# WinnerBy/PreGANPlus

Hardware: AMD Instinct MI355X
Metric: host-windows/sec (detect+diagnose+generate) (higher is better)
Workload: dtype fp32; 1 GPU; C2: PreGAN+ batched inference, 50 hosts x W=3 x 3 resources, 65536 windows per GPU, fp32; windows_per_gpu=65536, parallelism=dp1 (independent windows)

## Files before the change

### include/preganplus.h

```cpp
#ifndef PREGANPLUS_H
#define PREGANPLUS_H

#include <stddef.h>

#ifdef __cplusplus
extern "C" {
#endif

#define PGP_ABI_VERSION 1

#define PGP_OK 0
#define PGP_ERR_ARG (-1)
#define PGP_ERR_UNSUPPORTED (-2)
#define PGP_ERR_HIP (-3)
#define PGP_ERR_STATE (-4)

typedef struct pgp_model pgp_model;

int pgp_abi_version(void);
const char* pgp_last_error(void);

int pgp_supported_hosts(int* out, int cap);

int pgp_create(int n_hosts, int n_protos, pgp_model** out);
int pgp_destroy(pgp_model* m);

size_t pgp_weight_blob_len(int n_hosts, int n_protos);

int pgp_load_weights(pgp_model* m, const double* blob, size_t len);

int pgp_reserve(pgp_model* m, int max_batch);

int pgp_forward(pgp_model* m, int batch, const float* windows, const float* sched,
                float* logits, float* protos, int* cls, int* any_anom,
                float* probs, int* keep_orig, int* final_target, int* gen_target,
                float* latent, void* stream);

int pgp_forward_stage(pgp_model* m, int stage, int batch, const float* windows,
                      const float* sched, float* logits, float* protos, int* cls,
                      int* any_anom, float* probs, int* keep_orig, int* final_target,
                      int* gen_target, float* latent, void* stream);

int pgp_migrations(int n_hosts, int batch, const int* keep_orig, const int* final_target, const int* cur_host,
                   int* moves, int* hosts_from, void* stream);
int pgp_embedding(int n_hosts, int batch, const float* logits, const float* protos, float* emb, void* stream);
int pgp_decoder_split(pgp_model* m, int on);
int pgp_encoder_split(pgp_model* m, int on);
int pgp_gan_split(pgp_model* m, int on);
int pgp_schedule_onehot(int n_hosts, int batch, const unsigned char* idx, float* sched, void* stream);

int pgp_create_fpe(int n_hosts, pgp_model** out);
size_t pgp_fpe_weight_blob_len(int n_hosts);
int pgp_forward_fpe(pgp_model* m, int batch, const float* windows, const float* h0, const float* sched,
                    float* scores, float* protos, int* cls, int* any_anom, float* probs, int* keep_orig,
                    int* final_target, int* gen_target, void* stream);
int pgp_forward_fpe_stage(pgp_model* m, int stage, int batch, const float* windows, const float* h0,
                          const float* sched, float* scores, float* protos, int* cls, int* any_anom, float* probs,
                          int* keep_orig, int* final_target, int* gen_target, void* stream);

size_t pgp_master_len(int n_hosts);
size_t pgp_tune_workspace_len(int n_hosts, int batch);
size_t pgp_gan_workspace_len(int n_hosts, int batch);
size_t pgp_master_offset(int n_hosts, int section);

int pgp_tune_forward(int n_hosts, int batch, const float* windows, const float* P, float* workspace,
                     float* latent, float* logits, float* protos, void* stream);
int pgp_tune_backward(int n_hosts, int batch, const float* P, float* G, float* workspace, const float* logits,
                      const float* protos, const int* y, const float* mult, const float* tgt, void* stream);
int pgp_tune_backward_prefix(int n_hosts, int fwd_batch, int batch, const float* P, float* G, float* workspace,
                             const float* logits, const float* protos, const int* y, const float* mult,
                             const float* tgt, void* stream);
int pgp_tune_set_side_stream(void* stream);
int pgp_tune_reserve_cus(int n);
int pgp_tune_timing(int on);
int pgp_tune_fused_ms(float* ms6);
int pgp_tune_plan_info(int n_hosts, int fwd_batch, int batch, int* out, int cap);
int pgp_gan_plan_info(int n_hosts, int batch);
int pgp_tune_targets(int n_hosts, int n_protos, const float* logits, const float* protos, const int* y, const int* cls,
                     double* state, double update_min, double decay, float* mult, float* tgt, double* loss,
                     void* stream);
int pgp_tune_step1(int n_hosts, int n_protos, const float* window, const int* y, const int* cls, const float* P,
                   float* G, double* state, double update_min, double decay, float* logits, float* protos,
                   double* loss, void* stream);
size_t pgp_tune_dropout_mask_len(int n_hosts);
int pgp_tune_step1_dropout(int n_hosts, int n_protos, const float* window, const int* y, const int* cls,
                           const float* P, float* G, double* state, double update_min, double decay, float* logits,
                           float* protos, double* loss, float p, const unsigned long long* rng_device, int step,
                           void* stream);
int pgp_tune_dropout_masks(int n_hosts, float p, const unsigned long long* rng_device, int step, unsigned char* keep,
                           void* stream);
int pgp_tune_forward_many(int n_hosts, int n_windows, const float* windows, const float* P, double* logits,
                          double* protos, void* stream);
int pgp_forward1(int n_hosts, int n_protos, const float* window, const float* sched, const float* P,
                 const double* prototypes_device, float* logits, float* protos, int* cls, int* any_anom, float* probs,
                 int* keep_orig, int* final_target, int* gen_target, void* stream);
int pgp_tune_dataset(int n_hosts, int n_env, int n_rows, const double* series, const double* train_max,
                     float* windows, int* y, int* cls, float* infer, void* stream);
size_t pgp_tune_targets_dp_workspace_len(int batch);
int pgp_tune_targets_dp(int n_hosts, int n_protos, int batch, const float* logits, const float* protos, const int* y,
                        const int* cls, const double* state, double update_min, float* mult, float* tgt, double* loss,
                        double* inc, double* workspace, void* stream);
int pgp_tune_state_apply(int n_protos, double* state, const double* inc, double decay, int n_cond,
                         const int* cond_rows, double* cond_steps, float* adam_table, double lr, double beta1,
                         double beta2, void* stream);
int pgp_gan_forward(int n_hosts, int batch, const float* emb, const float* sched, const float* P, float* workspace,
                    float* ns, float* probs, void* stream);
int pgp_gan_disc_backward(int n_hosts, int batch, const float* target, const float* P, float* G, float* workspace,
                          void* stream);
int pgp_gan_gen_backward(int n_hosts, int batch, const float* P, float* G, float* workspace, void* stream);
int pgp_gan_probs(int n_hosts, int batch, const float* workspace, float* probs, void* stream);

typedef struct {
  long long offset;
  int n;
  int active;
  float step_size;
  float bc2_sqrt;
} pgp_adam_tensor;
int pgp_adamw(float* P, const float* G, float* exp_avg, float* exp_avg_sq, float lr, float weight_decay,
              float beta1, float beta2, float eps, const pgp_adam_tensor* tensors, int ntensors, void* stream);
int pgp_adamw_table(float* P, const float* G, float* exp_avg, float* exp_avg_sq, float lr, float weight_decay,
                    float beta1, float beta2, float eps, const pgp_adam_tensor* tensors, int ntensors,
                    const float* sched, void* stream);

int pgp_gan_forward1(int n_hosts, const float* emb, const float* sched, const float* P, float* workspace, float* ns,
                     float* probs, void* stream);
int pgp_gan_step1(int n_hosts, const float* target, float* P, float* G, float* exp_avg, float* exp_avg_sq,
                  float lr_disc, float lr_gen, float weight_decay, float beta1, float beta2, float eps,
                  const pgp_adam_tensor* disc_tensors, int n_disc, const float* disc_sched,
                  const pgp_adam_tensor* gen_tensors, int n_gen, const float* gen_sched, float* workspace,
                  float* probs_gen, float* probs_after, void* stream);

typedef struct {
  long long offset;
  int n;
  int section;
  int cond;
  double step;
} pgp_online_tensor;
typedef struct {
  int n_hosts, n_env, n_rows, n_protos;
  const double* series;
  const double* train_max;
  const float* sched;
  const double* envs;
  float *P, *G, *exp_avg, *exp_avg_sq;
  float* tune_ws;
  float *logits, *protos, *windows;
  int *y, *cls;
  double* state;
  float *mult, *tgt;
  double *loss, *inc, *dp_ws;
  float* adam_rows;
  double* cond_steps;
  float *gan_ws, *ns, *probs, *emb;
  double* sim_out;
  float* target;
  const pgp_online_tensor* tensors;
  int n_tensors, n_cond;
  double lr[3];
  double weight_decay, beta1, beta2, eps, update_min, decay;
} pgp_online_desc;
typedef struct pgp_online pgp_online;
typedef int (*pgp_collective_fn)(void* user, int which, void* stream);
#define PGP_COLL_DISC_GRAD 0
#define PGP_COLL_GEN_GRAD 1
#define PGP_COLL_TUNE_GRAD 2
#define PGP_COLL_TUNE_STATE 3
#define PGP_ONLINE_NSTAGE 10
int pgp_online_create(const pgp_online_desc* desc, pgp_online** out);
int pgp_online_destroy(pgp_online* h);
int pgp_online_step(pgp_online* h, void* main_stream, void* gan_stream, pgp_collective_fn cb, void* user);
int pgp_online_timing(pgp_online* h, int on);
int pgp_online_issue_worker(pgp_online* h, int on);
int pgp_online_stage_ms(pgp_online* h, float* ms);
int pgp_online_steps(const pgp_online* h, double* steps, int n);
int pgp_online_gan_step(pgp_online* h, void* stream);

size_t pgp_fpe_param_len(int n_hosts);
int pgp_fpe_train_step(int n_hosts, int n_protos, const float* window, const float* h0, const int* y, const int* cls,
                       const float* P, float* G, double* state, double update_min, double decay, double* loss,
                       void* stream);
int pgp_fpe_forward_many(int n_hosts, int n, const float* windows, const float* h0, const float* P, double* probs,
                         double* protos, void* stream);

int pgp_load_weights_master(pgp_model* m, const float* P_device, const double* prototypes);
int pgp_repack_master(pgp_model* m, const float* P_device, const double* prototypes_device, void* stream);
int pgp_repack_master_sections(pgp_model* m, const float* P_device, const double* prototypes_device, int sections,
                               void* stream);

typedef struct pgp_gobi pgp_gobi;
size_t pgp_gobi_weight_len(int n_hosts);
int pgp_gobi_create(int n_hosts, const float* weights, size_t len, pgp_gobi** out);
int pgp_gobi_destroy(pgp_gobi* g);
const char* pgp_gobi_last_error(void);
int pgp_gobi_optimize(pgp_gobi* g, int n_env, const float* init, float* result, int* iterations,
                      float* fitness, int max_iters, float* pre, void* stream);

int pgp_gobi_train_steps(int n_hosts, int n_samples, int n, const float* feats, const float* targets,
                         const int* order, float* P, float* exp_avg, float* exp_avg_sq, long long step0,
                         double lr, double weight_decay, double beta1, double beta2, double eps, float* loss,
                         void* stream);
int pgp_gobi_train_eval(int n_hosts, int n_samples, int n, const float* feats, const float* targets,
                        const int* order, const float* P, float* loss, void* stream);

typedef struct pgp_gobi_job {
  long long sample_off, order_off;
  long long step0;
  int n_samples, n;
  double lr, weight_decay, beta1, beta2, eps;
} pgp_gobi_job;
int pgp_gobi_train_steps_many(int n_hosts, int n_models, const pgp_gobi_job* jobs, long long n_pool_samples,
                              const float* feats, const float* targets, long long n_pool_steps, const int* order,
                              float* P, float* exp_avg, float* exp_avg_sq, float* loss, void* jobs_dev,
                              void* stream);
int pgp_gobi_train_eval_many(int n_hosts, int n_models, const pgp_gobi_job* jobs, long long n_pool_samples,
                             const float* feats, const float* targets, long long n_pool_steps, const int* order,
                             const float* P, float* loss, void* jobs_dev, void* stream);

int pgp_gobi_create_many(int n_hosts, int n_models, const float* weights, size_t len, pgp_gobi** out);
int pgp_gobi_model_count(const pgp_gobi* g);
int pgp_gobi_set_model(pgp_gobi* g, int m, const float* weights, size_t len);
int pgp_gobi_optimize_groups(pgp_gobi* g, int n_env, int n_groups, const int* groups, const float* init,
                             float* result, int* iterations, float* fitness, int max_iters, float* pre,
                             void* stream);
int pgp_gobi_plan_groups(int n_env, const int* model_of_env, int n_models, int* groups_out, int cap);

size_t pgp_sim_env_len(int n_hosts);
int pgp_simulate(int n_hosts, int n_env, const double* envs, const float* new_sched, const float* orig_sched,
                 double* out, float* target, void* stream);

#ifdef __cplusplus
}
#endif

#endif
```

### preganplus_amd/_native.py

```python
from __future__ import annotations

import ctypes
import os

_HERE = os.path.dirname(os.path.abspath(__file__))
LIB_PATH = os.environ.get("PGP_LIB", os.path.join(_HERE, "_lib", "libpreganplus.so"))

PGP_OK = 0
_ERRS = {-1: "PGP_ERR_ARG", -2: "PGP_ERR_UNSUPPORTED", -3: "PGP_ERR_HIP", -4: "PGP_ERR_STATE"}

_lib = None

REMOVED_ENV = ("PGP_TUNE_SIDE_STREAM", "PGP_TUNE_SIDE_MIN_TOKENS", "PGP_TUNE_DEC_DWS", "PGP_TUNE_SIDE_EARLY",
               "PGP_TUNE_EARLY_FLUSH", "PGP_TF_SPREAD", "PGP_C3_GAN_LATE", "PGP_INIT_SEED", "PGP_SAVE_GAN_INTERVAL")


def _warn_removed_env():
    import warnings
    for k in REMOVED_ENV:
        if k in os.environ:
            hint = " (use the init_seed argument)" if k == "PGP_INIT_SEED" else ""
            warnings.warn(f"{k} is no longer read by preganplus_amd{hint}; it has no effect", RuntimeWarning,
                          stacklevel=3)


class NativeError(RuntimeError):
    pass


def lib():
    global _lib
    if _lib is not None:
        return _lib
    _warn_removed_env()
    if not os.path.exists(LIB_PATH):
        raise ImportError(
            f"HIP library not found at {LIB_PATH}; build it with `make` "
            "(hipcc --offload-arch=gfx950). There is no CPU fallback.")
    L = ctypes.CDLL(LIB_PATH)
    c_int, c_size, vp = ctypes.c_int, ctypes.c_size_t, ctypes.c_void_p
    fp = ctypes.c_void_p
    L.pgp_abi_version.argtypes = []
    L.pgp_abi_version.restype = c_int
    L.pgp_last_error.argtypes = []
    L.pgp_last_error.restype = ctypes.c_char_p
    L.pgp_supported_hosts.argtypes = [ctypes.POINTER(c_int), c_int]
    L.pgp_supported_hosts.restype = c_int
    L.pgp_weight_blob_len.argtypes = [c_int, c_int]
    L.pgp_weight_blob_len.restype = c_size
    L.pgp_create.argtypes = [c_int, c_int, ctypes.POINTER(vp)]
    L.pgp_create.restype = c_int
    L.pgp_destroy.argtypes = [vp]
    L.pgp_destroy.restype = c_int
    L.pgp_load_weights.argtypes = [vp, ctypes.POINTER(ctypes.c_double), c_size]
    L.pgp_load_weights.restype = c_int
    L.pgp_reserve.argtypes = [vp, c_int]
    L.pgp_reserve.restype = c_int
    L.pgp_forward.argtypes = [vp, c_int] + [fp] * 11 + [vp]
    L.pgp_forward.restype = c_int
    L.pgp_forward_stage.argtypes = [vp, c_int, c_int] + [fp] * 11 + [vp]
    L.pgp_forward_stage.restype = c_int
    L.pgp_create_fpe.argtypes = [c_int, ctypes.POINTER(vp)]
    L.pgp_create_fpe.restype = c_int
    L.pgp_fpe_weight_blob_len.argtypes = [c_int]
    L.pgp_fpe_weight_blob_len.restype = c_size
    L.pgp_forward_fpe.argtypes = [vp, c_int] + [fp] * 11 + [vp]
    L.pgp_forward_fpe.restype = c_int
    L.pgp_forward_fpe_stage.argtypes = [vp, c_int, c_int] + [fp] * 11 + [vp]
    L.pgp_forward_fpe_stage.restype = c_int
    L.pgp_migrations.argtypes = [c_int, c_int] + [fp] * 5 + [vp]
    L.pgp_migrations.restype = c_int
    L.pgp_embedding.argtypes = [c_int, c_int] + [fp] * 3 + [vp]
    L.pgp_embedding.restype = c_int
    L.pgp_decoder_split.argtypes = [vp, c_int]
    L.pgp_decoder_split.restype = c_int
    L.pgp_encoder_split.argtypes = [vp, c_int]
    L.pgp_encoder_split.restype = c_int
    L.pgp_gan_split.argtypes = [vp, c_int]
    L.pgp_gan_split.restype = c_int
    L.pgp_schedule_onehot.argtypes = [c_int, c_int, fp, fp, vp]
    L.pgp_schedule_onehot.restype = c_int
    _lib = L
    return L


def check(rc, what=""):
    if rc != PGP_OK:
        msg = lib().pgp_last_error().decode(errors="replace")
        raise NativeError(f"{what}: {_ERRS.get(rc, rc)}: {msg}")


def supported_hosts():
    buf = (ctypes.c_int * 16)()
    n = lib().pgp_supported_hosts(buf, 16)
    return [buf[i] for i in range(n)]
```

### preganplus_amd/csrc/pgp_capi.hip

```cpp
#include <hip/hip_runtime.h>

#include <string>

#include "../../include/preganplus.h"
#include "pgp_device.hpp"
#include "pgp_pack.hpp"
#include "pgp_repack.hpp"
#include "pgp_train.hpp"
#include "pgp_tune.hpp"
#include "pgp_tunef.hpp"
#include "pgp_tunedp.hpp"

#include <vector>

using namespace pgp;

struct pgp_model {
  int H = 0, K = 0;
  bool fpe = false;
  bool loaded = false;
  float* d_frags = nullptr;
  float* d_decb = nullptr;
  float* d_encb = nullptr;
  bool enc_split = true;
  bool dec_split = true;
  float* d_ganb = nullptr;
  bool gan_split = true;
  float* d_tab = nullptr;
  float* d_gtab = nullptr;
  float* d_gat = nullptr;
  double* d_pscr = nullptr;
  int cap = 0;
  float* d_agg = nullptr;
  float* d_lat = nullptr;
  float* d_emb = nullptr;
};

namespace {
thread_local std::string g_err;
int fail(int code, const std::string& msg) {
  g_err = msg;
  return code;
}
#define HIPCHK(x)                                                                                  \
  do {                                                                                             \
    hipError_t e_ = (x);                                                                           \
    if (e_ != hipSuccess) return fail(PGP_ERR_HIP, std::string(#x) + ": " + hipGetErrorString(e_)); \
  } while (0)

bool supported(int H) {
  switch (H) {
#define CASE(h) case h:
    PGP_FOR_EACH_H(CASE)
#undef CASE
    return true;
  }
  return false;
}

long lat_blk(int H) {
  switch (H) {
#define CASE(h) \
  case h:       \
    return Geo<h>::LAT_BLK;
    PGP_FOR_EACH_H(CASE)
#undef CASE
  }
  return 0;
}

int reserve(pgp_model* m, int n) {
  if (n <= m->cap) return PGP_OK;
  for (float** p : {&m->d_agg, &m->d_lat, &m->d_emb})
    if (*p) {
      HIPCHK(hipFree(*p));
      *p = nullptr;
    }
  m->cap = 0;
  const size_t nblk = (size_t)(n + 15) / 16;
  const size_t agg_f = m->fpe ? 4 : nblk * m->H * 3 * 48;
  const size_t lat_f = m->fpe ? 4 : nblk * (size_t)lat_blk(m->H);
  const size_t emb_f = nblk * 16 * round_up(2 * m->H, 16);
  HIPCHK(hipMalloc(&m->d_agg, agg_f * sizeof(float)));
  HIPCHK(hipMalloc(&m->d_lat, lat_f * sizeof(float)));
  HIPCHK(hipMalloc(&m->d_emb, emb_f * sizeof(float)));
  HIPCHK(hipMemset(m->d_agg, 0, agg_f * sizeof(float)));
  HIPCHK(hipMemset(m->d_lat, 0, lat_f * sizeof(float)));
  HIPCHK(hipMemset(m->d_emb, 0, emb_f * sizeof(float)));
  m->cap = n;
  return PGP_OK;
}
}

int pgp::set_error(int code, const std::string& msg) { return fail(code, msg); }

extern "C" {

int pgp_abi_version(void) { return PGP_ABI_VERSION; }
const char* pgp_last_error(void) { return g_err.c_str(); }

int pgp_supported_hosts(int* out, int cap) {
  int n = 0;
#define CASE(h)                         \
  if (out && n < cap) out[n] = h;       \
  ++n;
  PGP_FOR_EACH_H(CASE)
#undef CASE
  return n;
}

size_t pgp_weight_blob_len(int n_hosts, int n_protos) {
  if (!supported(n_hosts) || n_protos < 1) return 0;
  return blob_len(n_hosts, n_protos);
}

int pgp_create(int n_hosts, int n_protos, pgp_model** out) {
  if (!out) return fail(PGP_ERR_ARG, "out is NULL");
  *out = nullptr;
  if (!supported(n_hosts)) return fail(PGP_ERR_UNSUPPORTED, "host count not compiled in: " + std::to_string(n_hosts));
  if (n_protos < 1 || n_protos > kMaxProtos) return fail(PGP_ERR_ARG, "n_protos out of range [1,64]");
  pgp_model* m = new pgp_model();
  m->H = n_hosts;
  m->K = n_protos;
  *out = m;
  return PGP_OK;
}

size_t pgp_fpe_weight_blob_len(int n_hosts) { return fpe_blob_len(n_hosts); }

int pgp_create_fpe(int n_hosts, pgp_model** out) {
  if (!out) return fail(PGP_ERR_ARG, "out is NULL");
  *out = nullptr;
  if (fpe_blob_len(n_hosts) == 0)
    return fail(PGP_ERR_UNSUPPORTED, "FPE variant: host count not compiled in: " + std::to_string(n_hosts));
  pgp_model* m = new pgp_model();
  m->H = n_hosts;
  m->K = 3;
  m->fpe = true;
  *out = m;
  return PGP_OK;
}

int pgp_destroy(pgp_model* m) {
  if (!m) return PGP_OK;
  for (float* p : {m->d_frags, m->d_decb, m->d_encb, m->d_ganb, m->d_tab, m->d_gtab, m->d_agg, m->d_lat, m->d_emb, m->d_gat})
    if (p) (void)hipFree(p);
  if (m->d_pscr) (void)hipFree(m->d_pscr);
  delete m;
  return PGP_OK;
}

int pgp_load_weights(pgp_model* m, const double* blob, size_t len) {
  if (!m || !blob) return fail(PGP_ERR_ARG, "NULL model or blob");
  Packed P;
  const std::string err = m->fpe ? pack_fpe_weights(m->H, blob, len, &P) : pack_weights(m->H, m->K, blob, len, &P);
  if (!err.empty()) return fail(PGP_ERR_ARG, err);
  if (!m->d_frags) HIPCHK(hipMalloc(&m->d_frags, P.frags.size() * sizeof(float)));
  if (!m->d_tab) HIPCHK(hipMalloc(&m->d_tab, P.enc_tab.size() * sizeof(float)));
  if (!m->d_gtab) HIPCHK(hipMalloc(&m->d_gtab, P.gan_tab.size() * sizeof(float)));
  HIPCHK(hipMemcpy(m->d_frags, P.frags.data(), P.frags.size() * sizeof(float), hipMemcpyHostToDevice));
  HIPCHK(hipMemcpy(m->d_tab, P.enc_tab.data(), P.enc_tab.size() * sizeof(float), hipMemcpyHostToDevice));
  HIPCHK(hipMemcpy(m->d_gtab, P.gan_tab.data(), P.gan_tab.size() * sizeof(float), hipMemcpyHostToDevice));
  if (!m->d_gat) HIPCHK(hipMalloc(&m->d_gat, sizeof(GatConst)));
  HIPCHK(hipMemcpy(m->d_gat, &P.gat, sizeof(GatConst), hipMemcpyHostToDevice));
  if (!m->fpe && decoder_split_floats(m->H) > 0) {
    if (!m->d_decb) HIPCHK(hipMalloc(&m->d_decb, decoder_split_floats(m->H) * sizeof(float)));
    HIPCHK(launch_decoder_split(m->H, m->d_frags, m->d_decb, nullptr));
    HIPCHK(hipStreamSynchronize(nullptr));
  }
  if (!m->fpe && encoder_split_floats(m->H) > 0) {
    if (!m->d_encb) HIPCHK(hipMalloc(&m->d_encb, encoder_split_floats(m->H) * sizeof(float)));
    HIPCHK(launch_encoder_split(m->H, m->d_frags, m->d_encb, nullptr));
    HIPCHK(hipStreamSynchronize(nullptr));
  }
  if (gan_split_floats(m->H) > 0) {
    if (!m->d_ganb) HIPCHK(hipMalloc(&m->d_ganb, gan_split_floats(m->H) * sizeof(float)));
    HIPCHK(launch_gan_split_derive(m->H, m->d_frags, m->d_ganb, nullptr));
    HIPCHK(hipStreamSynchronize(nullptr));
  }
  m->loaded = true;
  return PGP_OK;
}

int pgp_reserve(pgp_model* m, int max_batch) {
  if (!m || max_batch < 0) return fail(PGP_ERR_ARG, "bad reserve arguments");
  return reserve(m, max_batch);
}

int pgp_forward_stage(pgp_model* m, int stage, int batch, const float* windows, const float* sched, float* logits,
                      float* protos, int* cls, int* any_anom, float* probs, int* keep_orig, int* final_target,
                      int* gen_target, float* latent, void* stream) {
  if (!m) return fail(PGP_ERR_ARG, "NULL model");
  if (!m->loaded) return fail(PGP_ERR_STATE, "weights not loaded");
  if (m->fpe) return fail(PGP_ERR_STATE, "FPE model: use pgp_forward_fpe");
  if (batch < 0) return fail(PGP_ERR_ARG, "negative batch");
  if (stage < -1 || stage > 3) return fail(PGP_ERR_ARG, "bad stage");
  if (batch == 0) return PGP_OK;
  const bool all = stage == -1;
  if (((all || stage == 0) && !windows) ||
      ((all || stage == 2) && (!logits || !protos || !cls || !any_anom)) ||
      ((all || stage == 3) && (!sched || !probs || !keep_orig || !final_target || !gen_target)))
    return fail(PGP_ERR_ARG, "NULL input/output pointer");
  if (batch > m->cap) {
    const int rc = reserve(m, batch);
    if (rc) return rc;
  }
  FwdArgs a{};
  a.B = batch;
  a.H = m->H;
  a.K = m->K;
  a.windows = windows;
  a.sched = sched;
  a.agg = m->d_agg;
  a.lat = m->d_lat;
  a.emb = m->d_emb;
  a.frags = m->d_frags;
  a.decb = m->dec_split ? m->d_decb : nullptr;
  a.encb = m->enc_split ? m->d_encb : nullptr;
  a.ganb = m->gan_split ? m->d_ganb : nullptr;
  a.tab = m->d_tab;
  a.gtab = m->d_gtab;
  a.gat = m->d_gat;
  a.logits = logits;
  a.protos = protos;
  a.cls = cls;
  a.any_anom = any_anom;
  a.probs = probs;
  a.keep = keep_orig;
  a.final_t = final_target;
  a.gen_t = gen_target;
  a.latent = latent;
  hipStream_t st = reinterpret_cast<hipStream_t>(stream);
  if (all || stage == 0) HIPCHK(launch_gat(a, st));
  if (all || stage == 1) HIPCHK(launch_encoder(a, st));
  if (all || stage == 2) HIPCHK(launch_decoder(a, st));
  if (all || stage == 3) HIPCHK(launch_gan(a, st));
  return PGP_OK;
}

int pgp_forward(pgp_model* m, int batch, const float* windows, const float* sched, float* logits, float* protos,
                int* cls, int* any_anom, float* probs, int* keep_orig, int* final_target, int* gen_target,
                float* latent, void* stream) {
  return pgp_forward_stage(m, -1, batch, windows, sched, logits, protos, cls, any_anom, probs, keep_orig,
                           final_target, gen_target, latent, stream);
}

int pgp_forward_fpe_stage(pgp_model* m, int stage, int batch, const float* windows, const float* h0,
                          const float* sched, float* scores, float* protos, int* cls, int* any_anom, float* probs,
                          int* keep_orig, int* final_target, int* gen_target, void* stream) {
  if (!m) return fail(PGP_ERR_ARG, "NULL model");
  if (!m->loaded) return fail(PGP_ERR_STATE, "weights not loaded");
  if (!m->fpe) return fail(PGP_ERR_STATE, "not an FPE model: use pgp_forward");
  if (batch < 0) return fail(PGP_ERR_ARG, "negative batch");
  if (stage < -1 || stage > 1) return fail(PGP_ERR_ARG, "bad stage");
  if (batch == 0) return PGP_OK;
  const bool all = stage == -1;
  if (((all || stage == 0) && (!windows || !h0 || !scores || !protos || !cls || !any_anom)) ||
      ((all || stage == 1) && (!sched || !probs || !keep_orig || !final_target || !gen_target)))
    return fail(PGP_ERR_ARG, "NULL input/output pointer");
  if (batch > m->cap) {
    const int rc = reserve(m, batch);
    if (rc) return rc;
  }
  hipStream_t st = reinterpret_cast<hipStream_t>(stream);
  FpeArgs f{};
  f.B = batch;
  f.windows = windows;
  f.h0 = h0;
  f.tab = m->d_tab;
  f.scores = scores;
  f.protos = protos;
  f.cls = cls;
  f.any_anom = any_anom;
  f.emb = m->d_emb;
  if (all || stage == 0) HIPCHK(launch_fpe(m->H, f, st));
  FwdArgs a{};
  a.B = batch;
  a.H = m->H;
  a.K = m->K;
  a.sched = sched;
  a.emb = m->d_emb;
  a.frags = m->d_frags;
  a.ganb = m->gan_split ? m->d_ganb : nullptr;
  a.gtab = m->d_gtab;
  a.probs = probs;
  a.keep = keep_orig;
  a.final_t = final_target;
  a.gen_t = gen_target;
  if (all || stage == 1) HIPCHK(launch_gan(a, st));
  return PGP_OK;
}

int pgp_forward_fpe(pgp_model* m, int batch, const float* windows, const float* h0, const float* sched,
                    float* scores, float* protos, int* cls, int* any_anom, float* probs, int* keep_orig,
                    int* final_target, int* gen_target, void* stream) {
  return pgp_forward_fpe_stage(m, -1, batch, windows, h0, sched, scores, protos, cls, any_anom, probs, keep_orig,
                               final_target, gen_target, stream);
}

int pgp_migrations(int n_hosts, int batch, const int* keep_orig, const int* final_target, const int* cur_host,
                   int* moves, int* hosts_from, void* stream) {
  if (n_hosts < 1 || batch < 0) return fail(PGP_ERR_ARG, "bad migrations arguments");
  if (batch == 0) return PGP_OK;
  if (!keep_orig || !final_target || !cur_host || !moves || !hosts_from)
    return fail(PGP_ERR_ARG, "NULL input/output pointer");
  HIPCHK(launch_decide(batch, n_hosts, keep_orig, final_target, cur_host, moves, hosts_from,
                       reinterpret_cast<hipStream_t>(stream)));
  return PGP_OK;
}

int pgp_embedding(int n_hosts, int batch, const float* logits, const float* protos, float* emb, void* stream) {
  if (n_hosts < 1 || batch < 0) return fail(PGP_ERR_ARG, "bad embedding arguments");
  if (batch == 0) return PGP_OK;
  if (!logits || !protos || !emb) return fail(PGP_ERR_ARG, "NULL input/output pointer");
  HIPCHK(launch_embed((long)batch * n_hosts, logits, protos, emb, reinterpret_cast<hipStream_t>(stream)));
  return PGP_OK;
}

int pgp_decoder_split(pgp_model* m, int on) {
  if (!m) return fail(PGP_ERR_ARG, "NULL model");
  if (m->fpe || decoder_split_floats(m->H) == 0)
    return on ? fail(PGP_ERR_UNSUPPORTED, "split-bf16 decoder not compiled for this model / host count") : PGP_OK;
  m->dec_split = on != 0;
  return PGP_OK;
}

int pgp_encoder_split(pgp_model* m, int on) {
  if (!m) return fail(PGP_ERR_ARG, "NULL model");
  if (m->fpe || encoder_split_floats(m->H) == 0)
    return on ? fail(PGP_ERR_UNSUPPORTED, "split-bf16 encoder not compiled for this model / host count") : PGP_OK;
  m->enc_split = on != 0;
  return PGP_OK;
}

int pgp_gan_split(pgp_model* m, int on) {
  if (!m) return fail(PGP_ERR_ARG, "NULL model");
  if (gan_split_floats(m->H) == 0)
    return on ? fail(PGP_ERR_UNSUPPORTED, "split-bf16 GAN kernel not compiled for this host count") : PGP_OK;
  m->gan_split = on != 0;
  return PGP_OK;
}

int pgp_schedule_onehot(int n_hosts, int batch, const unsigned char* idx, float* sched, void* stream) {
  if (n_hosts < 1 || n_hosts > 255 || batch < 0) return fail(PGP_ERR_ARG, "bad schedule_onehot arguments");
  if (batch == 0) return PGP_OK;
  if (!idx || !sched) return fail(PGP_ERR_ARG, "NULL input/output pointer");
  HIPCHK(launch_onehot(n_hosts, (long)batch * n_hosts, idx, sched, reinterpret_cast<hipStream_t>(stream)));
  return PGP_OK;
}

namespace {
bool master_offsets(int H, long* tr, long* gen, long* disc, long* all) {
  switch (H) {
#define CASE(h)                     \
  case h:                           \
    *tr = 0;                        \
    *gen = TGeo<h>::OFF_GEN;        \
    *disc = TGeo<h>::OFF_DISC;      \
    *all = TGeo<h>::ALL;            \
    return true;
    PGP_FOR_EACH_H(CASE)
#undef CASE
  }
  return false;
}
}

size_t pgp_master_len(int n_hosts) {
  long a, b, c, d;
  return master_offsets(n_hosts, &a, &b, &c, &d) ? (size_t)d : 0;
}
size_t pgp_master_offset(int n_hosts, int section) {
  long a, b, c, d;
  if (!master_offsets(n_hosts, &a, &b, &c, &d)) return 0;
  return section == 0 ? a : section == 1 ? b : section == 2 ? c : d;
}
size_t pgp_tune_workspace_len(int n_hosts, int batch) {
  TunePlan p;
  return (supported(n_hosts) && tune_plan(n_hosts, batch, &p)) ? (size_t)p.total : 0;
}
size_t pgp_gan_workspace_len(int n_hosts, int batch) {
  return supported(n_hosts) ? (size_t)gan_workspace_floats(n_hosts, batch) : 0;
}

int pgp_tune_forward(int n_hosts, int batch, const float* windows, const float* P, float* workspace, float* latent,
                     float* logits, float* protos, void* stream) {
  if (!supported(n_hosts)) return fail(PGP_ERR_UNSUPPORTED, "host count");
  if (batch < 0 || (batch > 0 && (!windows || !P || !workspace || !logits || !protos)))
    return fail(PGP_ERR_ARG, "bad tune_forward arguments");
  if (batch == 0) return PGP_OK;
  TunePlan p;
  tune_plan(n_hosts, batch, &p);
  HIPCHK(launch_tune_forward(p, windows, P, workspace, latent, logits, protos, reinterpret_cast<hipStream_t>(stream)));
  return PGP_OK;
}

int pgp_tune_backward(int n_hosts, int batch, const float* P, float* G, float* workspace, const float* logits,
                      const float* protos, const int* y, const float* mult, const float* tgt, void* stream) {
  if (!supported(n_hosts)) return fail(PGP_ERR_UNSUPPORTED, "host count");
  if (batch < 0 || (batch > 0 && (!P || !G || !workspace || !logits || !protos || !y || !mult || !tgt)))
    return fail(PGP_ERR_ARG, "bad tune_backward arguments");
  if (batch == 0) return PGP_OK;
  TunePlan p;
  tune_plan(n_hosts, batch, &p);
  HIPCHK(launch_tune_backward(p, P, G, workspace, logits, protos, y, mult, tgt,
                              reinterpret_cast<hipStream_t>(stream)));
  return PGP_OK;
}

int pgp_tune_backward_prefix(int n_hosts, int fwd_batch, int batch, const float* P, float* G, float* workspace,
                             const float* logits, const float* protos, const int* y, const float* mult,
                             const float* tgt, void* stream) {
  if (!supported(n_hosts)) return fail(PGP_ERR_UNSUPPORTED, "host count");
  if (batch < 0 || batch > fwd_batch ||
      (batch > 0 && (!P || !G || !workspace || !logits || !protos || !y || !mult || !tgt)))
    return fail(PGP_ERR_ARG, "bad tune_backward_prefix arguments");
  if (batch == 0) return PGP_OK;
  TunePlan p;
  if (!tune_plan_prefix(n_hosts, fwd_batch, batch, &p)) return fail(PGP_ERR_ARG, "tune_backward_prefix plan");
  HIPCHK(launch_tune_backward(p, P, G, workspace, logits, protos, y, mult, tgt,
                              reinterpret_cast<hipStream_t>(stream)));
  return PGP_OK;
}

size_t pgp_fpe_param_len(int n_hosts) { return (size_t)fpe_param_count(n_hosts); }

static const char* kFpeTrainHosts = "FPE training: n_hosts 16 or 50 only (FPE_16's architecture)";

int pgp_fpe_train_step(int n_hosts, int n_protos, const float* window, const float* h0, const int* y, const int* cls,
                       const float* P, float* G, double* state, double update_min, double decay, double* loss,
                       void* stream) {
  if (fpe_param_count(n_hosts) == 0) return fail(PGP_ERR_UNSUPPORTED, kFpeTrainHosts);
  if (n_protos < 3 || n_protos > kMaxProtos) return fail(PGP_ERR_ARG, "n_protos");
  if (!window || !h0 || !y || !cls || !P || !G || !state || !loss) return fail(PGP_ERR_ARG, "NULL argument");
  HIPCHK(launch_fpe_step(n_hosts, window, h0, y, cls, P, G, n_protos, state, update_min, decay, loss,
                         reinterpret_cast<hipStream_t>(stream)));
  return PGP_OK;
}

int pgp_fpe_forward_many(int n_hosts, int n, const float* windows, const float* h0, const float* P, double* probs,
                         double* protos, void* stream) {
  if (fpe_param_count(n_hosts) == 0) return fail(PGP_ERR_UNSUPPORTED, kFpeTrainHosts);
  if (n < 0 || (n > 0 && (!windows || !h0 || !P || !probs || !protos))) return fail(PGP_ERR_ARG, "bad arguments");
  if (n == 0) return PGP_OK;
  HIPCHK(launch_fpe_forward_many(n_hosts, n, windows, h0, P, probs, protos, reinterpret_cast<hipStream_t>(stream)));
  return PGP_OK;
}

static const char* kGobiTrainHosts = "GOBI surrogate training: only energy_latency_16 exists (16 hosts)";

int pgp_gobi_train_steps(int n_hosts, int n_samples, int n, const float* feats, const float* targets,
                         const int* order, float* P, float* exp_avg, float* exp_avg_sq, long long step0,
                         double lr, double weight_decay, double beta1, double beta2, double eps, float* loss,
                         void* stream) {
  if (!gobi_train_supported(n_hosts)) return fail(PGP_ERR_UNSUPPORTED, kGobiTrainHosts);
  if (n < 0 || n_samples < 0 || step0 < 0)
    return fail(PGP_ERR_ARG, "gobi_train_steps: negative n, n_samples or step0");
  if (!(lr > 0.0) || !(weight_decay >= 0.0) || !(eps >= 0.0) || !(beta1 >= 0.0 && beta1 < 1.0) ||
      !(beta2 >= 0.0 && beta2 < 1.0))
    return fail(PGP_ERR_ARG, "gobi_train_steps: lr > 0, weight_decay >= 0, eps >= 0, betas in [0, 1)");
  if (n == 0) return PGP_OK;
  if (!feats || !targets || !order || !P || !exp_avg || !exp_avg_sq || !loss)
    return fail(PGP_ERR_ARG, "gobi_train_steps: NULL argument");
  const GobiTrainHyper hy{lr, weight_decay, beta1, beta2, eps};
  HIPCHK(launch_gobi_train_steps(n_hosts, n_samples, n, feats, targets, order, P, exp_avg, exp_avg_sq, step0, hy,
                                 loss, reinterpret_cast<hipStream_t>(stream)));
  return PGP_OK;
}

int pgp_gobi_train_eval(int n_hosts, int n_samples, int n, const float* feats, const float* targets, const int* order,
                        const float* P, float* loss, void* stream) {
  if (!gobi_train_supported(n_hosts)) return fail(PGP_ERR_UNSUPPORTED, kGobiTrainHosts);
  if (n < 0 || n_samples < 0) return fail(PGP_ERR_ARG, "gobi_train_eval: negative n or n_samples");
  if (n == 0) return PGP_OK;
  if (!feats || !targets || !order || !P || !loss) return fail(PGP_ERR_ARG, "gobi_train_eval: NULL argument");
  HIPCHK(launch_gobi_train_eval(n_hosts, n_samples, n, feats, targets, order, P, loss,
                                reinterpret_cast<hipStream_t>(stream)));
  return PGP_OK;
}

namespace {
int gobi_jobs_check(const char* who, bool steps, int n_hosts, int n_models, const pgp_gobi_job* jobs,
                    long long n_pool_samples, long long n_pool_steps, bool* work, int* max_n) {
  const std::string w(who);
  *work = false;
  *max_n = 0;
  if (!gobi_train_supported(n_hosts)) return fail(PGP_ERR_UNSUPPORTED, kGobiTrainHosts);
  if (n_models < 0 || n_pool_samples < 0 || n_pool_steps < 0)
    return fail(PGP_ERR_ARG, w + ": negative n_models or pool size");
  if (n_models == 0) return PGP_OK;
  if (!jobs) return fail(PGP_ERR_ARG, w + ": NULL jobs");
  for (int m = 0; m < n_models; ++m) {
    const pgp_gobi_job& j = jobs[m];
    const std::string at = w + ": job " + std::to_string(m) + ": ";
    if (j.n < 0 || j.n_samples < 0 || (steps && j.step0 < 0))
      return fail(PGP_ERR_ARG, at + "negative n, n_samples or step0");
    if (steps && (!(j.lr > 0.0) || !(j.weight_decay >= 0.0) || !(j.eps >= 0.0) ||
                  !(j.beta1 >= 0.0 && j.beta1 < 1.0) || !(j.beta2 >= 0.0 && j.beta2 < 1.0)))
      return fail(PGP_ERR_ARG, at + "lr > 0, weight_decay >= 0, eps >= 0, betas in [0, 1)");
    if (j.sample_off < 0 || j.sample_off > n_pool_samples || j.n_samples > n_pool_samples - j.sample_off)
      return fail(PGP_ERR_ARG, at + "sample range outside the pool");
    if (j.order_off < 0 || j.order_off > n_pool_steps || j.n > n_pool_steps - j.order_off)
      return fail(PGP_ERR_ARG, at + "order / loss range outside the pool");
    if (j.n > 0) *work = true;
    if (j.n > *max_n) *max_n = j.n;
  }
  return PGP_OK;
}
}

int pgp_gobi_train_steps_many(int n_hosts, int n_models, const pgp_gobi_job* jobs, long long n_pool_samples,
                              const float* feats, const float* targets, long long n_pool_steps, const int* order,
                              float* P, float* exp_avg, float* exp_avg_sq, float* loss, void* jobs_dev,
                              void* stream) {
  bool work;
  int max_n;
  const int rc = gobi_jobs_check("gobi_train_steps_many", true, n_hosts, n_models, jobs, n_pool_samples,
                                 n_pool_steps, &work, &max_n);
  if (rc != PGP_OK || !work) return rc;
  if (!feats || !targets || !order || !P || !exp_avg || !exp_avg_sq || !loss || !jobs_dev)
    return fail(PGP_ERR_ARG, "gobi_train_steps_many: NULL argument");
  hipStream_t st = reinterpret_cast<hipStream_t>(stream);
  HIPCHK(hipMemcpyAsync(jobs_dev, jobs, (size_t)n_models * sizeof(pgp_gobi_job), hipMemcpyHostToDevice, st));
  HIPCHK(launch_gobi_train_steps_many(n_hosts, n_models, static_cast<const pgp_gobi_job*>(jobs_dev), feats, targets,
                                      order, P, exp_avg, exp_avg_sq, loss, st));
  return PGP_OK;
}

int pgp_gobi_train_eval_many(int n_hosts, int n_models, const pgp_gobi_job* jobs, long long n_pool_samples,
                             const float* feats, const float* targets, long long n_pool_steps, const int* order,
                             const float* P, float* loss, void* jobs_dev, void* stream) {
  bool work;
  int max_n;
  const int rc = gobi_jobs_check("gobi_train_eval_many", false, n_hosts, n_models, jobs, n_pool_samples,
                                 n_pool_steps, &work, &max_n);
  if (rc != PGP_OK || !work) return rc;
  if (!feats || !targets || !order || !P || !loss || !jobs_dev)
    return fail(PGP_ERR_ARG, "gobi_train_eval_many: NULL argument");
  hipStream_t st = reinterpret_cast<hipStream_t>(stream);
  HIPCHK(hipMemcpyAsync(jobs_dev, jobs, (size_t)n_models * sizeof(pgp_gobi_job), hipMemcpyHostToDevice, st));
  HIPCHK(launch_gobi_train_eval_many(n_hosts, n_models, max_n, static_cast<const pgp_gobi_job*>(jobs_dev), feats,
                                     targets, order, P, loss, st));
  return PGP_OK;
}

int pgp_tune_reserve_cus(int n) {
  if (n < 0) return fail(PGP_ERR_ARG, "negative CU count");
  tf_reserve_cus(n);
  return PGP_OK;
}

int pgp_tune_set_side_stream(void* stream) {
  HIPCHK(tune_set_side_stream(reinterpret_cast<hipStream_t>(stream)));
  return PGP_OK;
}

int pgp_tune_timing(int on) {
  HIPCHK(tune_timing(on != 0));
  return PGP_OK;
}

int pgp_tune_plan_info(int n_hosts, int fwd_batch, int batch, int* out, int cap) {
  if (!supported(n_hosts)) return fail(PGP_ERR_UNSUPPORTED, "host count");
  if (!out || cap < 0 || batch < 1 || batch > fwd_batch) return fail(PGP_ERR_ARG, "bad tune_plan_info arguments");
  int v[kTunePlanInfo];
  if (!tune_plan_info(n_hosts, fwd_batch, batch, v)) return fail(PGP_ERR_ARG, "tune_plan_info plan");
  for (int i = 0; i < kTunePlanInfo && i < cap; ++i) out[i] = v[i];
  return kTunePlanInfo;
}

int pgp_gan_plan_info(int n_hosts, int batch) {
  if (!supported(n_hosts)) return fail(PGP_ERR_UNSUPPORTED, "host count");
  if (batch < 1) return fail(PGP_ERR_ARG, "batch >= 1");
  const int s = gan_plan_slices(n_hosts, batch);
  return s > 0 ? s : fail(PGP_ERR_UNSUPPORTED, "host count");
}

int pgp_tune_fused_ms(float* ms6) {
  if (!ms6) return fail(PGP_ERR_ARG, "NULL output");
  const hipError_t e = tune_fused_ms(ms6);
  if (e == hipErrorInvalidValue) return fail(PGP_ERR_STATE, "pgp_tune_timing(1) was never called");
  HIPCHK(e);
  return PGP_OK;
}

int pgp_tune_targets(int n_hosts, int n_protos, const float* logits, const float* protos, const int* y, const int* cls,
                     double* state, double update_min, double decay, float* mult, float* tgt, double* loss,
                     void* stream) {
  if (n_hosts <= 0 || n_hosts > 64) return fail(PGP_ERR_UNSUPPORTED, "host count");
  if (n_protos < 3) return fail(PGP_ERR_ARG, "triplet_loss needs prototypes 0-2");
  if (!logits || !protos || !y || !cls || !state || !mult || !tgt || !loss)
    return fail(PGP_ERR_ARG, "bad tune_targets arguments");
  HIPCHK(launch_tune_targets(n_hosts, n_protos, logits, protos, y, cls, state, update_min, decay, mult, tgt, loss,
                             reinterpret_cast<hipStream_t>(stream)));
  return PGP_OK;
}

int pgp_tune_step1(int n_hosts, int n_protos, const float* window, const int* y, const int* cls, const float* P,
                   float* G, double* state, double update_min, double decay, float* logits, float* protos,
                   double* loss, void* stream) {
  if (!tune1_supported(n_hosts)) return fail(PGP_ERR_UNSUPPORTED, "host count (fused step: 8 or 16)");
  if (n_protos < 3) return fail(PGP_ERR_ARG, "triplet_loss needs prototypes 0-2");
  if (!window || !y || !cls || !P || !G || !state || !logits || !protos || !loss)
    return fail(PGP_ERR_ARG, "bad tune_step1 arguments");
  HIPCHK(launch_tune1(n_hosts, n_protos, window, y, cls, P, G, state, update_min, decay, logits, protos, loss,
                      reinterpret_cast<hipStream_t>(stream)));
  return PGP_OK;
}

size_t pgp_tune_dropout_mask_len(int n_hosts) { return tune1_dropout_mask_len(n_hosts); }

namespace {
inline bool drop_threshold(float p, unsigned int* thr) {
  if (!(p >= 0.f && p < 1.f)) return false;
  *thr = (unsigned int)((double)p * 4294967296.0);
  return true;
}
}

int pgp_tune_step1_dropout(int n_hosts, int n_protos, const float* window, const int* y, const int* cls, const float* P,
                           float* G, double* state, double update_min, double decay, float* logits, float* protos,
                           double* loss, float p, const unsigned long long* rng_device, int step, void* stream) {
  if (!tune1_supported(n_hosts)) return fail(PGP_ERR_UNSUPPORTED, "host count (fused step with dropout: 8 or 16)");
  unsigned int thr = 0;
  if (!drop_threshold(p, &thr)) return fail(PGP_ERR_ARG, "dropout p outside [0, 1)");
  if (n_protos < 3) return fail(PGP_ERR_ARG, "triplet_loss needs prototypes 0-2");
  if (!window || !y || !cls || !P || !G || !state || !logits || !protos || !loss || step < 0)
    return fail(PGP_ERR_ARG, "bad tune_step1_dropout arguments");
  hipStream_t st = reinterpret_cast<hipStream_t>(stream);
  if (thr == 0) {
    HIPCHK(launch_tune1(n_hosts, n_protos, window, y, cls, P, G, state, update_min, decay, logits, protos, loss, st));
    return PGP_OK;
  }
  if (!rng_device) return fail(PGP_ERR_ARG, "dropout needs rng_device = {seed, base step}");
  HIPCHK(launch_tune1_dropout(n_hosts, n_protos, window, y, cls, P, G, state, update_min, decay, logits, protos, loss,
                              thr, 1.0f / (1.0f - p), rng_device, step, st));
  return PGP_OK;
}

int pgp_tune_dropout_masks(int n_hosts, float p, const unsigned long long* rng_device, int step, unsigned char* keep,
                           void* stream) {
  if (!tune1_supported(n_hosts)) return fail(PGP_ERR_UNSUPPORTED, "host count (dropout masks: 8 or 16)");
  unsigned int thr = 0;
  if (!drop_threshold(p, &thr)) return fail(PGP_ERR_ARG, "dropout p outside [0, 1)");
  if (!rng_device || !keep || step < 0 || (reinterpret_cast<uintptr_t>(keep) & 3))
    return fail(PGP_ERR_ARG, "bad tune_dropout_masks arguments (keep: 4-byte aligned)");
  HIPCHK(launch_drop_masks(n_hosts, thr, rng_device, step, keep, reinterpret_cast<hipStream_t>(stream)));
  return PGP_OK;
}

int pgp_tune_forward_many(int n_hosts, int n_windows, const float* windows, const float* P, double* logits,
                          double* protos, void* stream) {
  if (!tune1_supported(n_hosts)) return fail(PGP_ERR_UNSUPPORTED, "host count (fused forward: 8 or 16)");
  if (n_windows < 0) return fail(PGP_ERR_ARG, "n_windows >= 0");
  if (n_windows == 0) return PGP_OK;
  if (!windows || !P || !logits || !protos) return fail(PGP_ERR_ARG, "bad tune_forward_many arguments");
  HIPCHK(launch_fwd_many(n_hosts, n_windows, windows, P, logits, protos, reinterpret_cast<hipStream_t>(stream)));
  return PGP_OK;
}

int pgp_forward1(int n_hosts, int n_protos, const float* window, const float* sched, const float* P,
                 const double* prototypes_device, float* logits, float* protos, int* cls, int* any_anom, float* probs,
                 int* keep_orig, int* final_target, int* gen_target, void* stream) {
  if (!tune1_supported(n_hosts)) return fail(PGP_ERR_UNSUPPORTED, "host count (batch-1 forward: 8 or 16)");
  if (n_protos < 1 || n_protos > kMaxProtos) return fail(PGP_ERR_ARG, "n_protos out of range");
  if (!window || !sched || !P || !prototypes_device || !logits || !protos || !cls || !any_anom || !probs ||
      !keep_orig || !final_target || !gen_target)
    return fail(PGP_ERR_ARG, "bad forward1 arguments");
  HIPCHK(launch_infer1(n_hosts, n_protos, window, sched, P, prototypes_device, logits, protos, cls, any_anom, probs,
                       keep_orig, final_target, gen_target, reinterpret_cast<hipStream_t>(stream)));
  return PGP_OK;
}

int pgp_tune_dataset(int n_hosts, int n_env, int n_rows, const double* series, const double* train_max,
                     float* windows, int* y, int* cls, float* infer, void* stream) {
  if (n_hosts <= 0 || n_hosts > 64) return fail(PGP_ERR_UNSUPPORTED, "host count");
  if (n_env < 0 || n_rows < 1 || n_rows > kMaxTuneRows) return fail(PGP_ERR_ARG, "n_env >= 0, 1 <= n_rows <= 16");
  if (n_env == 0) return PGP_OK;
  if (!series || !train_max || !windows || !y || !cls) return fail(PGP_ERR_ARG, "bad tune_dataset arguments");
  HIPCHK(launch_tune_dataset(n_hosts, n_env, n_rows, series, train_max, windows, y, cls, infer,
                             reinterpret_cast<hipStream_t>(stream)));
  return PGP_OK;
}

size_t pgp_tune_targets_dp_workspace_len(int batch) {
  return batch > 0 ? (size_t)tune_dp_workspace_doubles(batch) : 0;
}

int pgp_tune_targets_dp(int n_hosts, int n_protos, int batch, const float* logits, const float* protos, const int* y,
                        const int* cls, const double* state, double update_min, float* mult, float* tgt, double* loss,
                        double* inc, double* workspace, void* stream) {
  if (n_hosts <= 0 || n_hosts > 64) return fail(PGP_ERR_UNSUPPORTED, "host count");
  if (n_protos < 3 || n_protos > kMaxProtos) return fail(PGP_ERR_ARG, "triplet_loss needs prototypes 0-2");
  if (batch <= 0 || !logits || !protos || !y || !cls || !state || !mult || !tgt || !loss || !inc || !workspace)
    return fail(PGP_ERR_ARG, "bad tune_targets_dp arguments");
  HIPCHK(launch_tune_targets_dp(n_hosts, n_protos, batch, logits, protos, y, cls, const_cast<double*>(state),
                                update_min, mult, tgt, loss, inc, workspace, reinterpret_cast<hipStream_t>(stream)));
  return PGP_OK;
}

int pgp_tune_state_apply(int n_protos, double* state, const double* inc, double decay, int n_cond,
                         const int* cond_rows, double* cond_steps, float* adam_table, double lr, double beta1,
                         double beta2, void* stream) {
  if (n_protos < 3 || n_protos > kMaxProtos || !state || !inc) return fail(PGP_ERR_ARG, "bad state arguments");
  if (n_cond < 0 || n_cond > kMaxCond || (n_cond > 0 && (!cond_rows || !cond_steps || !adam_table)))
    return fail(PGP_ERR_ARG, "bad AdamW condition arguments");
  CondRows cr{};
  cr.n = n_cond;
  for (int i = 0; i < n_cond; ++i) {
    if (cond_rows[i] < 0 || cond_rows[i] >= kMaxTensors) return fail(PGP_ERR_ARG, "AdamW table row out of range");
    cr.row[i] = cond_rows[i];
  }
  HIPCHK(launch_tune_state_apply(n_protos, state, inc, decay, cr, cond_steps, adam_table, lr, beta1, beta2,
                                 reinterpret_cast<hipStream_t>(stream)));
  return PGP_OK;
}

int pgp_gan_forward(int n_hosts, int batch, const float* emb, const float* sched, const float* P, float* workspace,
                    float* ns, float* probs, void* stream) {
  long tr, go, dof, all;
  if (!master_offsets(n_hosts, &tr, &go, &dof, &all)) return fail(PGP_ERR_UNSUPPORTED, "host count");
  if (batch < 0 || (batch > 0 && (!emb || !sched || !P || !workspace || !ns || !probs)))
    return fail(PGP_ERR_ARG, "bad gan_forward arguments");
  if (batch == 0) return PGP_OK;
  HIPCHK(launch_gan_fwd(n_hosts, batch, emb, sched, P + go, P + dof, workspace, ns, probs,
                        reinterpret_cast<hipStream_t>(stream)));
  return PGP_OK;
}

int pgp_gan_disc_backward(int n_hosts, int batch, const float* target, const float* P, float* G, float* workspace,
                          void* stream) {
  long tr, go, dof, all;
  if (!master_offsets(n_hosts, &tr, &go, &dof, &all)) return fail(PGP_ERR_UNSUPPORTED, "host count");
  if (batch < 0 || (batch > 0 && (!target || !P || !G || !workspace))) return fail(PGP_ERR_ARG, "bad arguments");
  if (batch == 0) return PGP_OK;
  HIPCHK(launch_gan_disc_bwd(n_hosts, batch, target, P + dof, G + dof, workspace,
                             reinterpret_cast<hipStream_t>(stream)));
  return PGP_OK;
}

int pgp_gan_gen_backward(int n_hosts, int batch, const float* P, float* G, float* workspace, void* stream) {
  long tr, go, dof, all;
  if (!master_offsets(n_hosts, &tr, &go, &dof, &all)) return fail(PGP_ERR_UNSUPPORTED, "host count");
  if (batch < 0 || (batch > 0 && (!P || !G || !workspace))) return fail(PGP_ERR_ARG, "bad arguments");
  if (batch == 0) return PGP_OK;
  HIPCHK(launch_gan_gen_bwd(n_hosts, batch, P + go, P + dof, G + go, workspace,
                            reinterpret_cast<hipStream_t>(stream)));
  return PGP_OK;
}

int pgp_gan_forward1(int n_hosts, const float* emb, const float* sched, const float* P, float* workspace, float* ns,
                     float* probs, void* stream) {
  long tr, go, dof, all;
  if (!gan1_supported(n_hosts) || !master_offsets(n_hosts, &tr, &go, &dof, &all))
    return fail(PGP_ERR_UNSUPPORTED, "host count (fused GAN step: 8 or 16)");
  if (!emb || !sched || !P || !workspace || !ns || !probs) return fail(PGP_ERR_ARG, "bad gan_forward1 arguments");
  HIPCHK(launch_gan1_forward(n_hosts, emb, sched, P + go, P + dof, workspace, ns, probs,
                             reinterpret_cast<hipStream_t>(stream)));
  return PGP_OK;
}

static bool adam_args(AdamArgs* a, float* P, float* G, float* m, float* v, float lr, float wd, float b1, float b2,
                      float eps, const pgp_adam_tensor* t, int n, const float* sched, long lo, long hi) {
  if (!t || !sched || n < 0 || n > kMaxTensors) return false;
  *a = AdamArgs{};
  a->param = P;
  a->grad = G;
  a->m = m;
  a->v = v;
  a->lr_wd = lr * wd;
  a->b1 = b1;
  a->b2 = b2;
  a->eps = eps;
  a->ntensors = n;
  a->sched = sched;
  for (int i = 0; i < n; ++i) {
    if (t[i].offset < lo || t[i].n < 0 || (long)t[i].offset + t[i].n > hi) return false;
    a->t[i].off = (long)t[i].offset;
    a->t[i].n = t[i].n;
    a->t[i].active = 1;
  }
  return true;
}

int pgp_gan_step1(int n_hosts, const float* target, float* P, float* G, float* exp_avg, float* exp_avg_sq,
                  float lr_disc, float lr_gen, float weight_decay, float beta1, float beta2, float eps,
                  const pgp_adam_tensor* disc_tensors, int n_disc, const float* disc_sched,
                  const pgp_adam_tensor* gen_tensors, int n_gen, const float* gen_sched, float* workspace,
                  float* probs_gen, float* probs_after, void* stream) {
  long tr, go, dof, all;
  if (!gan1_supported(n_hosts) || !master_offsets(n_hosts, &tr, &go, &dof, &all))
    return fail(PGP_ERR_UNSUPPORTED, "host count (fused GAN step: 8 or 16)");
  if (!target || !P || !G || !exp_avg || !exp_avg_sq || !workspace || !probs_gen || !probs_after)
    return fail(PGP_ERR_ARG, "bad gan_step1 arguments");
  AdamArgs ad, ag;
  if (!adam_args(&ad, P, G, exp_avg, exp_avg_sq, lr_disc, weight_decay, beta1, beta2, eps, disc_tensors, n_disc,
                 disc_sched, dof, all) ||
      !adam_args(&ag, P, G, exp_avg, exp_avg_sq, lr_gen, weight_decay, beta1, beta2, eps, gen_tensors, n_gen,
                 gen_sched, go, dof))
    return fail(PGP_ERR_ARG, "AdamW tensors (disc / gen sections) or tables");
  HIPCHK(launch_gan1_step(n_hosts, target, P + go, P + dof, G + go, G + dof, workspace, ad, ag, probs_gen, probs_after,
                          reinterpret_cast<hipStream_t>(stream)));
  return PGP_OK;
}

int pgp_gan_probs(int n_hosts, int batch, const float* workspace, float* probs, void* stream) {
  if (!supported(n_hosts)) return fail(PGP_ERR_UNSUPPORTED, "host count");
  if (batch < 0 || (batch > 0 && (!workspace || !probs))) return fail(PGP_ERR_ARG, "bad arguments");
  if (batch == 0) return PGP_OK;
  HIPCHK(launch_gan_probs(n_hosts, batch, workspace, probs, reinterpret_cast<hipStream_t>(stream)));
  return PGP_OK;
}

int pgp_adamw(float* P, const float* G, float* exp_avg, float* exp_avg_sq, float lr, float weight_decay,
              float beta1, float beta2, float eps, const pgp_adam_tensor* tensors, int ntensors, void* stream) {
  if (!P || !G || !exp_avg || !exp_avg_sq || !tensors || ntensors < 0 || ntensors > kMaxTensors)
    return fail(PGP_ERR_ARG, "bad adamw arguments");
  if (ntensors == 0) return PGP_OK;
  AdamArgs a{};
  a.param = P;
  a.grad = const_cast<float*>(G);
  a.m = exp_avg;
  a.v = exp_avg_sq;
  a.lr_wd = lr * weight_decay;
  a.b1 = beta1;
  a.b2 = beta2;
  a.eps = eps;
  a.ntensors = ntensors;
  for (int i = 0; i < ntensors; ++i) {
    a.t[i].off = (long)tensors[i].offset;
    a.t[i].n = tensors[i].n;
    a.t[i].active = tensors[i].active;
    a.t[i].step_size = tensors[i].step_size;
    a.t[i].bc2_sqrt = tensors[i].bc2_sqrt;
  }
  HIPCHK(launch_adamw(a, reinterpret_cast<hipStream_t>(stream)));
  return PGP_OK;
}

int pgp_adamw_table(float* P, const float* G, float* exp_avg, float* exp_avg_sq, float lr, float weight_decay,
                    float beta1, float beta2, float eps, const pgp_adam_tensor* tensors, int ntensors,
                    const float* sched, void* stream) {
  if (!P || !G || !exp_avg || !exp_avg_sq || !tensors || !sched || ntensors < 0 || ntensors > kMaxTensors)
    return fail(PGP_ERR_ARG, "bad adamw arguments");
  if (ntensors == 0) return PGP_OK;
  AdamArgs a{};
  a.param = P;
  a.grad = const_cast<float*>(G);
  a.m = exp_avg;
  a.v = exp_avg_sq;
  a.lr_wd = lr * weight_decay;
  a.b1 = beta1;
  a.b2 = beta2;
  a.eps = eps;
  a.ntensors = ntensors;
  a.sched = sched;
  for (int i = 0; i < ntensors; ++i) {
    a.t[i].off = (long)tensors[i].offset;
    a.t[i].n = tensors[i].n;
    a.t[i].active = kAdamFromTable;
    a.t[i].step_size = tensors[i].step_size;
    a.t[i].bc2_sqrt = tensors[i].bc2_sqrt;
  }
  HIPCHK(launch_adamw(a, reinterpret_cast<hipStream_t>(stream)));
  return PGP_OK;
}

int pgp_repack_master(pgp_model* m, const float* P_device, const double* prototypes_device, void* stream) {
  return pgp_repack_master_sections(m, P_device, prototypes_device, 3, stream);
}

int pgp_repack_master_sections(pgp_model* m, const float* P_device, const double* prototypes_device, int sections,
                               void* stream) {
  if (!m || !P_device || !prototypes_device) return fail(PGP_ERR_ARG, "NULL argument");
  if (sections < 1 || sections > 3) return fail(PGP_ERR_ARG, "sections: 1 (PreGAN+), 2 (GAN) or 3 (both)");
  if (m->fpe) return fail(PGP_ERR_STATE, "FPE model: master-layout reload covers the PreGAN+ model only");
  if (!m->loaded) return fail(PGP_ERR_STATE, "weights not loaded (the first load packs on the host)");
  long tr, go, dof, all;
  if (!master_offsets(m->H, &tr, &go, &dof, &all)) return fail(PGP_ERR_UNSUPPORTED, "host count");
  if (repack_blob_protos_offset(m->H, m->K) != all) return fail(PGP_ERR_STATE, "master / blob layout mismatch");
  if (!m->d_pscr) HIPCHK(hipMalloc(&m->d_pscr, repack_scratch_len(m->H) * sizeof(double)));
  RepackArgs a{m->K, P_device, all, prototypes_device, m->d_pscr, m->d_frags, m->d_tab, m->d_gtab, m->d_gat, sections};
  HIPCHK(launch_repack(m->H, a, reinterpret_cast<hipStream_t>(stream)));
  if ((sections & 1) && m->d_decb)
    HIPCHK(launch_decoder_split(m->H, m->d_frags, m->d_decb, reinterpret_cast<hipStream_t>(stream)));
  if ((sections & 1) && m->d_encb)
    HIPCHK(launch_encoder_split(m->H, m->d_frags, m->d_encb, reinterpret_cast<hipStream_t>(stream)));
  if ((sections & 2) && m->d_ganb)
    HIPCHK(launch_gan_split_derive(m->H, m->d_frags, m->d_ganb, reinterpret_cast<hipStream_t>(stream)));
  return PGP_OK;
}

int pgp_load_weights_master(pgp_model* m, const float* P_device, const double* prototypes) {
  if (!m || !P_device || !prototypes) return fail(PGP_ERR_ARG, "NULL argument");
  if (m->fpe) return fail(PGP_ERR_STATE, "FPE model: master-layout reload covers the PreGAN+ model only");
  long tr, go, dof, all;
  if (!master_offsets(m->H, &tr, &go, &dof, &all)) return fail(PGP_ERR_UNSUPPORTED, "host count");
  std::vector<float> host((size_t)all);
  HIPCHK(hipMemcpy(host.data(), P_device, host.size() * sizeof(float), hipMemcpyDeviceToHost));
  std::vector<double> blob(host.size() + 2 * (size_t)m->K);
  for (size_t i = 0; i < host.size(); ++i) blob[i] = host[i];
  for (int k = 0; k < 2 * m->K; ++k) blob[host.size() + k] = prototypes[k];
  return pgp_load_weights(m, blob.data(), blob.size());
}

}
```

### preganplus_amd/csrc/pgp_device.hpp

```cpp
#pragma once
#include <hip/hip_runtime.h>

#include <atomic>
#include <string>

#include "pgp_layout.hpp"

struct pgp_gobi_job;

namespace pgp {

typedef float f32x4 __attribute__((ext_vector_type(4)));
typedef float f32x2 __attribute__((ext_vector_type(2)));

constexpr int kMaxProtos = 64;

inline int device_cus() {
  static std::atomic<int> cached[64];
  int dev = 0;
  if (hipGetDevice(&dev) != hipSuccess || dev < 0 || dev >= 64) return 256;
  int n = cached[dev].load(std::memory_order_relaxed);
  if (n == 0) {
    if (hipDeviceGetAttribute(&n, hipDeviceAttributeMultiprocessorCount, dev) != hipSuccess || n <= 0) n = 256;
    cached[dev].store(n, std::memory_order_relaxed);
  }
  return n;
}

struct FwdArgs {
  int B, H, K;
  const float* windows;
  const float* sched;
  float* agg;
  float* lat;
  float* emb;
  const float* frags;
  const float* decb;
  const float* ganb;
  const float* encb;
  const float* tab;
  const float* gtab;
  const float* gat;
  float* logits;
  float* protos;
  int* cls;
  int* any_anom;
  float* probs;
  int* keep;
  int* final_t;
  int* gen_t;
  float* latent;
};

struct FpeArgs {
  int B;
  const float* windows;
  const float* h0;
  const float* tab;
  float* scores;
  float* protos;
  int* cls;
  int* any_anom;
  float* emb;
};
hipError_t launch_fpe(int H, const FpeArgs& a, hipStream_t st);
int fpe_param_count(int H);
hipError_t launch_fpe_step(int n_hosts, const float* win, const float* h0, const int* y, const int* cls,
                           const float* P, float* G, int K, double* state, double update_min, double decay,
                           double* loss, hipStream_t st);
hipError_t launch_fpe_forward_many(int n_hosts, int n, const float* wins, const float* h0s, const float* P,
                                   double* probs, double* protos, hipStream_t st);

struct GobiTrainHyper {
  double lr, wd, beta1, beta2, eps;
};
bool gobi_train_supported(int H);
hipError_t launch_gobi_train_steps(int n_hosts, int n_samples, int n, const float* feats, const float* targets,
                                   const int* order, float* P, float* m, float* v, long long step0,
                                   const GobiTrainHyper& hy, float* loss, hipStream_t st);
hipError_t launch_gobi_train_eval(int n_hosts, int n_samples, int n, const float* feats, const float* targets,
                                  const int* order, const float* P, float* loss, hipStream_t st);
hipError_t launch_gobi_train_steps_many(int n_hosts, int n_models, const pgp_gobi_job* jobs_dev, const float* feats,
                                        const float* targets, const int* order, float* P, float* m, float* v,
                                        float* loss, hipStream_t st);
hipError_t launch_gobi_train_eval_many(int n_hosts, int n_models, int max_n, const pgp_gobi_job* jobs_dev,
                                       const float* feats, const float* targets, const int* order, const float* P,
                                       float* loss, hipStream_t st);

hipError_t launch_decide(int B, int C, const int* keep, const int* target, const int* cur, int* moves,
                         int* hosts_from, hipStream_t st);
hipError_t launch_embed(long n, const float* logits, const float* protos, float* emb, hipStream_t st);
hipError_t launch_onehot(int H, long rows, const unsigned char* idx, float* sched, hipStream_t st);

hipError_t launch_gat(const FwdArgs& a, hipStream_t st);
hipError_t launch_encoder(const FwdArgs& a, hipStream_t st);
hipError_t launch_decoder(const FwdArgs& a, hipStream_t st);
long decoder_split_floats(int H);
hipError_t launch_decoder_split(int H, const float* frags, float* decb, hipStream_t st);
long encoder_split_floats(int H);
hipError_t launch_encoder_split(int H, const float* frags, float* encb, hipStream_t st);
hipError_t launch_gan(const FwdArgs& a, hipStream_t st);
long gan_split_floats(int H);
hipError_t launch_gan_split_derive(int H, const float* frags, float* planes, hipStream_t st);
hipError_t launch_gan_split(const FwdArgs& a, hipStream_t st);

struct AdamArgs;
struct AdamFuse;
long gan_workspace_floats(int H, int B);
int gan_plan_slices(int H, int B);
hipError_t launch_adamw(const AdamArgs& a, hipStream_t st);
bool gan1_supported(int H);
hipError_t launch_gan1_forward(int H, const float* emb, const float* sched, const float* Pg, const float* Pd,
                               float* row, float* ns, float* probs, hipStream_t st);
hipError_t launch_gan1_step(int H, const float* target, float* Pg, float* Pd, float* Gg, float* Gd, float* row,
                            const AdamArgs& ad, const AdamArgs& ag, float* probs_gen, float* probs_after,
                            hipStream_t st);

hipError_t launch_gan_fwd(int H, int B, const float* emb, const float* sched, const float* Pg, const float* Pd,
                          float* ws, float* ns_out, float* probs, hipStream_t st, const float* logits = nullptr,
                          const float* protos = nullptr, float* emb_out = nullptr);
hipError_t launch_gan_disc_bwd(int H, int B, const float* target, const float* Pd, float* Gdd, float* ws,
                               hipStream_t st, float* probs = nullptr, const AdamFuse* af = nullptr);
hipError_t launch_gan_gen_bwd(int H, int B, const float* Pg, const float* Pd, float* Gdg, float* ws,
                              hipStream_t st, const AdamFuse* af = nullptr);
hipError_t launch_gan_probs(int H, int B, const float* ws, float* probs, hipStream_t st);
hipError_t launch_simulate(int H, int E, const double* envs, const float* new_sched, const float* orig_sched,
                           double* out, float* target, hipStream_t st);

#define PGP_DEV __device__ __forceinline__

PGP_DEV f32x4 mfma(float a, float b, f32x4 c) { return __builtin_amdgcn_mfma_f32_16x16x4f32(a, b, c, 0, 0, 0); }
typedef __bf16 bf16x8 __attribute__((ext_vector_type(8)));
typedef unsigned u32x4 __attribute__((ext_vector_type(4)));
PGP_DEV unsigned bf16_bits(float x) {
  const unsigned u = __float_as_uint(x);
  return (u + 0x7FFFu + ((u >> 16) & 1u)) >> 16;
}
PGP_DEV float bf16_val(unsigned h) { return __uint_as_float(h << 16); }
typedef __bf16 bf16x2 __attribute__((ext_vector_type(2)));
PGP_DEV unsigned bf16_pack(f32x2 x) { return __builtin_bit_cast(unsigned, __builtin_convertvector(x, bf16x2)); }
PGP_DEV f32x2 bf16_unpack(unsigned h) { return f32x2{__uint_as_float(h << 16), __uint_as_float(h & 0xFFFF0000u)}; }
PGP_DEV void split8(const float (&v)[8], u32x4 (&p)[3]) {
#pragma unroll
  for (int d = 0; d < 4; ++d) {
    const f32x2 x = {v[2 * d], v[2 * d + 1]};
    const unsigned h0 = bf16_pack(x);
    const f32x2 r1 = x - bf16_unpack(h0);
    const unsigned h1 = bf16_pack(r1);
    const f32x2 r2 = r1 - bf16_unpack(h1);
    p[0][d] = h0;
    p[1][d] = h1;
    p[2][d] = bf16_pack(r2);
  }
}
PGP_DEV f32x4 mfma_bf(u32x4 a, u32x4 b, f32x4 c) {
  return __builtin_amdgcn_mfma_f32_16x16x32_bf16(__builtin_bit_cast(bf16x8, a), __builtin_bit_cast(bf16x8, b), c, 0,
                                                 0, 0);
}
PGP_DEV void planes_ready(const u32x4 (&w)[3]) { asm volatile("" ::"v"(w[0]), "v"(w[1]), "v"(w[2])); }
PGP_DEV f32x4 mfma_bf6(const u32x4 (&w)[3], const u32x4 (&x)[3], f32x4 c) {
  c = mfma_bf(w[2], x[0], c);
  c = mfma_bf(w[1], x[1], c);
  c = mfma_bf(w[0], x[2], c);
  c = mfma_bf(w[1], x[0], c);
  c = mfma_bf(w[0], x[1], c);
  return mfma_bf(w[0], x[0], c);
}
PGP_DEV f32x4 mfma_bf3(const u32x4 (&w)[3], const u32x4 (&x)[3], f32x4 c) {
  c = mfma_bf(w[2], x[0], c);
  c = mfma_bf(w[1], x[0], c);
  return mfma_bf(w[0], x[0], c);
}

PGP_DEV bool arrive_last(unsigned* ctr, unsigned n, int* flag) {
  asm volatile("s_waitcnt vmcnt(0)" ::: "memory");
  __syncthreads();
  if (threadIdx.x == 0) {
    const bool last = __hip_atomic_fetch_add(ctr, 1u, __ATOMIC_RELAXED, __HIP_MEMORY_SCOPE_AGENT) == n - 1;
    if (last) {
      __builtin_amdgcn_fence(__ATOMIC_ACQUIRE, "agent");
      asm volatile("s_waitcnt vmcnt(0)" ::: "memory");
      __hip_atomic_store(ctr, 0u, __ATOMIC_RELAXED, __HIP_MEMORY_SCOPE_AGENT);
    }
    *flag = last;
  }
  __syncthreads();
  return *flag != 0;
}
PGP_DEV void store_wt(float* p, float v) { __hip_atomic_store(p, v, __ATOMIC_RELAXED, __HIP_MEMORY_SCOPE_AGENT); }
PGP_DEV f32x4 ld4(const float* p) { return *reinterpret_cast<const f32x4*>(p); }
PGP_DEV float tanh_fast(float x) {
  const float e = __expf(2.f * x);
  return 1.f - 2.f * __builtin_amdgcn_rcpf(e + 1.f);
}

PGP_DEV float xsum(float v, bool both) {
  const unsigned u = __float_as_uint(v);
  const auto r = __builtin_amdgcn_permlane16_swap(u, u, false, false);
  v = __uint_as_float(r[0]) + __uint_as_float(r[1]);
  if (both) {
    const unsigned u2 = __float_as_uint(v);
    const auto q = __builtin_amdgcn_permlane32_swap(u2, u2, false, false);
    v = __uint_as_float(q[0]) + __uint_as_float(q[1]);
  }
  return v;
}

PGP_DEV float pl_sum16(float a, float b) {
  const auto r = __builtin_amdgcn_permlane16_swap(__float_as_uint(a), __float_as_uint(b), false, false);
  return __uint_as_float(r[0]) + __uint_as_float(r[1]);
}
PGP_DEV float pl_sum32(float a, float b) {
  const auto r = __builtin_amdgcn_permlane32_swap(__float_as_uint(a), __float_as_uint(b), false, false);
  return __uint_as_float(r[0]) + __uint_as_float(r[1]);
}
PGP_DEV void xsum2(float& a, float& b) {
  const float s = pl_sum16(a, b);
  const unsigned su = __float_as_uint(s);
  const auto q = __builtin_amdgcn_permlane32_swap(su, su, false, false);
  const float t = __uint_as_float(q[0]) + __uint_as_float(q[1]);
  const unsigned tu = __float_as_uint(t);
  const auto p = __builtin_amdgcn_permlane16_swap(tu, tu, false, false);
  a = __uint_as_float(p[0]);
  b = __uint_as_float(p[1]);
}
PGP_DEV void xsum2_half(float& a, float& b) {
  const unsigned su = __float_as_uint(pl_sum16(a, b));
  const auto p = __builtin_amdgcn_permlane16_swap(su, su, false, false);
  a = __uint_as_float(p[0]);
  b = __uint_as_float(p[1]);
}
template <int NR>
PGP_DEV float xsum_rows(const float (&v)[NR]) {
  static_assert(NR >= 1 && NR <= 4, "at most 4 rows");
  const float s01 = pl_sum16(v[0], NR > 1 ? v[1] : 0.f);
  const float s23 = NR > 2 ? pl_sum16(v[2], NR > 3 ? v[3] : 0.f) : 0.f;
  return pl_sum32(s01, s23);
}

PGP_DEV void dma_groups(const float* __restrict__ src, float* dst, int ngroups, int wv, int nwaves, int lane) {
  for (int g = wv; g < ngroups; g += nwaves) {
    unsigned off = (unsigned)lane * 16u;
    asm volatile("" : "+v"(off));
    __builtin_amdgcn_global_load_lds(
        (const __attribute__((address_space(1))) void*)(reinterpret_cast<const char*>(src + (long)g * 256) + off),
        (__attribute__((address_space(3))) void*)(dst + g * 256), 16, 0, 0);
  }
}

int set_error(int code, const std::string& msg);

}
```

### preganplus_amd/csrc/pgp_encoder.hip

```cpp
#include "pgp_device.hpp"

namespace pgp {
namespace {

constexpr int kEncWaves = 4;
constexpr int kEnc16Waves = 4, kEnc16EU = 2;
template <int H>
constexpr bool tail_res() { return Geo<H>::TAIL; }
constexpr int kEncTailWaves = 8;
template <int H>
constexpr int enc_waves() { return H <= 16 ? kEnc16Waves : tail_res<H>() ? kEncTailWaves : kEncWaves; }
template <int H>
constexpr int NW_STAGE() { return enc_waves<H>(); }

#ifndef PGP_ENC_PIPE
#define PGP_ENC_PIPE 1
#endif
constexpr bool kEncPipe = PGP_ENC_PIPE != 0;
#ifndef PGP_ENC_PIPE_F32
#define PGP_ENC_PIPE_F32 0
#endif
constexpr bool kEncPipeF32 = PGP_ENC_PIPE_F32 != 0;

template <int H>
struct EncS {
  using G = Geo<H>;
  static constexpr int NBD = cdiv(G::KQ_D, 2);
  static constexpr int NBF = G::KQ_F / 2;
  static constexpr int F1S = G::MT_F * NBD * 3;
  static constexpr int F2S = G::MT_X * NBF * 3;
  static constexpr int FFN = F1S + F2S;
  static constexpr int L0F = 0;
  static constexpr int L1A = FFN;
  static constexpr int L1F = L1A + G::P_F1;
  static constexpr int GROUPS = L1F + FFN;
  static constexpr int STREAM = GROUPS * G::FQ;
  static constexpr long SIZE = STREAM;
};

template <int H, bool SPLIT = false>
struct EncLds {
  static constexpr bool TRES = tail_res<H>();
  static constexpr int RES0 = TRES ? Geo<H>::st_begin(Geo<H>::NST - 1) : 0;
  static constexpr int STREAM = SPLIT ? EncS<H>::STREAM : (kLayers * Geo<H>::LAYER_G - RES0) * Geo<H>::FQ;
  static constexpr bool RESIDENT = TRES || STREAM * 4 <= 32 * 1024;
  static constexpr int SLOT = Geo<H>::SLOT_G * Geo<H>::FQ;
  static constexpr int TAB = Geo<H>::t_size(kMaxProtos);
  static constexpr int TOTAL = (RESIDENT ? STREAM : 2 * SLOT) + TAB;
  static constexpr bool UNITS = TRES;
};

template <int H>
constexpr bool enc_split() {
  return tail_res<H>() && EncLds<H, true>::TOTAL * 4 + enc_waves<H>() * 144 * 4 <= 160 * 1024;
}

template <int H>
__global__ __launch_bounds__(256) void enc_split_kernel(const float* __restrict__ enc, float* __restrict__ out) {
  using G = Geo<H>;
  using S = EncS<H>;
  constexpr int T1 = G::MT_F * S::NBD, T2 = G::MT_X * S::NBF, TL = T1 + T2;
  const long f = (long)blockIdx.x * 4 + (threadIdx.x >> 6);
  const int lane = threadIdx.x & 63;
  if (f >= 2 * TL + G::P_F1) return;
  if (f >= 2 * TL) {
    const long i = f - 2 * TL;
    *reinterpret_cast<f32x4*>(out + (S::L1A + i) * 256 + lane * 4) = ld4(enc + (G::LAYER_G + i) * 256 + lane * 4);
    return;
  }
  const int l = (int)(f / TL), t = (int)(f % TL);
  const float* src = enc + (long)(l * G::LAYER_G + G::P_F1) * 256;
  long q0, q1, dst;
  const long base = l == 0 ? S::L0F : S::L1F;
  if (t < T1) {
    const int c = t / S::NBD, b = t % S::NBD;
    q0 = c * G::KQ_D + 2 * b;
    q1 = 2 * b + 1 < G::KQ_D ? q0 + 1 : -1;
    dst = base + (long)t * 3;
  } else {
    const int u = t - T1, m = u / S::NBF, b = u % S::NBF;
    q0 = G::G_F1 + m * G::KQ_F + 2 * b;
    q1 = q0 + 1;
    dst = base + S::F1S + (long)u * 3;
  }
  float v[8];
  const f32x4 x0 = ld4(src + q0 * 256 + lane * 4);
  const f32x4 x1 = q1 >= 0 ? ld4(src + q1 * 256 + lane * 4) : f32x4{0.f, 0.f, 0.f, 0.f};
#pragma unroll
  for (int e = 0; e < 4; ++e) {
    v[e] = x0[e];
    v[4 + e] = x1[e];
  }
  u32x4 p[3];
  split8(v, p);
#pragma unroll
  for (int k = 0; k < 3; ++k) *reinterpret_cast<u32x4*>(out + (dst + k) * 256 + lane * 4) = p[k];
}

template <int NT>
PGP_DEV void pair_tiles(const f32x4 (&T)[NT][3], int b, int w, float (&v)[8]) {
#pragma unroll
  for (int e = 0; e < 4; ++e) {
    v[e] = 2 * b < NT ? T[2 * b][w][e] : 0.f;
    v[4 + e] = 2 * b + 1 < NT ? T[2 * b + 1][w][e] : 0.f;
  }
}
PGP_DEV void planes_lds(const float* F, int lane, u32x4 (&w)[3]) {
#pragma unroll
  for (int k = 0; k < 3; ++k) w[k] = *reinterpret_cast<const u32x4*>(F + k * 256 + lane * 4);
}

template <int H>
PGP_DEV float relu_enc(float x) {
  if constexpr (Geo<H>::P8 || Geo<H>::TAIL)
    return __int_as_float(max(__float_as_int(x), 0));
  else
    return fmaxf(x, 0.f);
}

PGP_DEV void prio_mfma() { __builtin_amdgcn_s_setprio(1); }
PGP_DEV void prio_valu() { __builtin_amdgcn_s_setprio(0); }

template <int NM, int KQ, int KS, int NB, int NMA = NM>
PGP_DEV void gemm3(f32x4 (&acc)[NMA][3], const float* A, const f32x4 (&Bx)[NB][3], int lane) {
  static_assert(NM <= NMA, "accumulator tiles");
  prio_mfma();
#pragma unroll
  for (int m = 0; m < NM; ++m)
#pragma unroll
    for (int q4 = 0; q4 < KQ; ++q4) {
      const f32x4 a = ld4(A + (m * KQ + q4) * 256 + lane * 4);
#pragma unroll
      for (int e = 0; e < 4; ++e)
        if (4 * q4 + e < KS) {
#pragma unroll
          for (int w = 0; w < 3; ++w) acc[m][w] = mfma(a[e], Bx[q4][w][e], acc[m][w]);
        }
    }
  prio_valu();
}

template <int NM, int KQ, int KS, int NB, int NMA, int NR>
PGP_DEV void gemm3_rows(f32x4 (&acc)[NMA][3], const float* A, const f32x4 (&Bx)[NB][3], int lane,
                        float (&racc)[NR][3], const float* RW, int g) {
  static_assert(NM <= NMA, "accumulator tiles");
  prio_mfma();
  f32x4 an = ld4(A + lane * 4);
#pragma unroll
  for (int m = 0; m < NM; ++m)
#pragma unroll
    for (int q4 = 0; q4 < KQ; ++q4) {
      f32x4 a;
      if constexpr (kEncPipeF32) {
        a = an;
        if (m * KQ + q4 + 1 < NM * KQ) an = ld4(A + (m * KQ + q4 + 1) * 256 + lane * 4);
        __builtin_amdgcn_sched_barrier(0);
      } else {
        a = ld4(A + (m * KQ + q4) * 256 + lane * 4);
      }
      f32x4 rw[NR];
      if (m == 0) {
#pragma unroll
        for (int n = 0; n < NR; ++n) rw[n] = ld4(RW + ((n * KQ + q4) * 4 + g) * 4);
      }
#pragma unroll
      for (int e = 0; e < 4; ++e)
        if (4 * q4 + e < KS) {
#pragma unroll
          for (int w = 0; w < 3; ++w) {
            acc[m][w] = mfma(a[e], Bx[q4][w][e], acc[m][w]);
            if (m == 0) {
#pragma unroll
              for (int n = 0; n < NR; ++n) racc[n][w] = fmaf(rw[n][e], Bx[q4][w][e], racc[n][w]);
            }
          }
        }
    }
  prio_valu();
}

template <int NR>
PGP_DEV void rows_finish(float (&r)[NR][3]) {
  float* f = &r[0][0];
#pragma unroll
  for (int i = 0; i + 1 < 3 * NR; i += 2) xsum2(f[i], f[i + 1]);
  if constexpr ((3 * NR) % 2) f[3 * NR - 1] = xsum(f[3 * NR - 1], true);
}

template <int NR>
PGP_DEV float rows_pick(const float (&r)[NR][3], int w) {
  float v[NR];
#pragma unroll
  for (int n = 0; n < NR; ++n) v[n] = r[n][w];
  return xsum_rows<NR>(v);
}

template <int NR>
PGP_DEV void zero_rows(float (&r)[NR][3]) {
#pragma unroll
  for (int n = 0; n < NR; ++n)
#pragma unroll
    for (int w = 0; w < 3; ++w) r[n][w] = 0.f;
}

template <int H, bool AFFINE = true>
PGP_DEV void layer_norm_tiles(f32x4 (&acc)[Geo<H>::MT_D][3], f32x4 (&X)[Geo<H>::MT_D][3], const float* gam,
                              const float* bet, int g) {
  using G = Geo<H>;
  constexpr float invH = 1.0f / (float)H;
  float sum[3], mean[3], var[3];
#pragma unroll
  for (int w = 0; w < 3; ++w) {
    sum[w] = 0.f;
    float sq = 0.f;
#pragma unroll
    for (int mt = 0; mt < G::MT_D; ++mt) {
      sum[w] += (acc[mt][w][0] + acc[mt][w][1]) + (acc[mt][w][2] + acc[mt][w][3]);
#pragma unroll
      for (int r = 0; r < 4; ++r) sq = fmaf(acc[mt][w][r], acc[mt][w][r], sq);
    }
    xsum2(sum[w], sq);
    mean[w] = sum[w] * invH;
    var[w] = fmaxf(fmaf(-mean[w], mean[w], sq * invH), 0.f);
  }
#pragma unroll
  for (int w = 0; w < 3; ++w) {
    const float rstd = __builtin_amdgcn_rsqf(var[w] + 1e-5f);
    const float nm = -mean[w] * rstd;
#pragma unroll
    for (int mt = 0; mt < G::MT_D; ++mt) {
      f32x4 xn;
#pragma unroll
      for (int r = 0; r < 4; ++r) xn[r] = fmaf(acc[mt][w][r], rstd, nm);
      if constexpr (AFFINE) {
        const f32x4 ga = ld4(gam + 16 * mt + 4 * g), be = ld4(bet + 16 * mt + 4 * g);
        X[mt][w] = xn * ga + be;
      } else {
        X[mt][w] = xn;
      }
    }
  }
}

template <int H, bool SPLIT = false>
struct Ring {
  using G = Geo<H>;
  static constexpr bool RES = EncLds<H, SPLIT>::RESIDENT;
  float* cur;
  float* nxt;
  const float* enc;
  int next;
  int last;
  int wv, lane;
  PGP_DEV void issue() {
    if constexpr (RES) return;
    if (next < last) {
      const int si = next % (kLayers * G::NST), l = si / G::NST, k = si % G::NST;
      dma_groups(enc + (long)(l * G::LAYER_G + G::st_begin(k)) * G::FQ, nxt, G::st_end(k) - G::st_begin(k), wv,
                 enc_waves<H>(), lane);
    }
  }
  PGP_DEV void advance() {
    if constexpr (RES) {
      const int si = next % (kLayers * G::NST), l = si / G::NST, k = si % G::NST;
      int gi;
      if constexpr (SPLIT)
        gi = l == 0 ? EncS<H>::L0F : k == 2 ? EncS<H>::L1F : EncS<H>::L1A + G::st_begin(k);
      else
        gi = l * G::LAYER_G + G::st_begin(k) - EncLds<H>::RES0;
      cur = nxt + (gi > 0 ? gi : 0) * G::FQ;
      ++next;
      __builtin_amdgcn_sched_barrier(0);
      return;
    }
    __syncthreads();
    float* t = cur;
    cur = nxt;
    nxt = t;
    ++next;
    issue();
  }
};

template <int H>
PGP_DEV void attention(const f32x4 (&QKV)[3 * Geo<H>::TP][3], f32x4 (&O)[Geo<H>::TP][3]) {
  using G = Geo<H>;
  float pr[3][3];
  float sc9[9];
#pragma unroll
  for (int i = 0; i < 9; ++i) {
    const int w = i / 3, w2 = i % 3;
    float part = 0.f;
#pragma unroll
    for (int tp = 0; tp < G::TP; ++tp)
#pragma unroll
      for (int r = 0; r < 4; ++r) part += QKV[tp][w][r] * QKV[G::TP + tp][w2][r];
    if constexpr (G::P8)
      sc9[i] = part;
    else
      sc9[i] = xsum(part, true);
  }
  if constexpr (G::P8) {
#pragma unroll
    for (int i = 0; i < 8; i += 2) xsum2_half(sc9[i], sc9[i + 1]);
    sc9[8] = xsum(sc9[8], false);
  }
#pragma unroll
  for (int w = 0; w < 3; ++w) {
    const float* sc = sc9 + 3 * w;
    const float m = fmaxf(sc[0], fmaxf(sc[1], sc[2]));
    const float e0 = __expf(sc[0] - m), e1 = __expf(sc[1] - m), e2 = __expf(sc[2] - m);
    const float inv = __builtin_amdgcn_rcpf(e0 + e1 + e2);
    pr[w][0] = e0 * inv;
    pr[w][1] = e1 * inv;
    pr[w][2] = e2 * inv;
  }
#pragma unroll
  for (int tp = 0; tp < G::TP; ++tp)
#pragma unroll
    for (int w = 0; w < 3; ++w)
      O[tp][w] = pr[w][0] * QKV[2 * G::TP + tp][0] + pr[w][1] * QKV[2 * G::TP + tp][1] +
                 pr[w][2] * QKV[2 * G::TP + tp][2];
}

template <int H>
PGP_DEV void qkv_gemm(f32x4 (&QKV)[3 * Geo<H>::TP][3], const float* A, const float* tabqkv,
                      const f32x4 (&X)[Geo<H>::MT_D][3], int lane, int g) {
  using G = Geo<H>;
#pragma unroll
  for (int m = 0; m < 3 * G::TP; ++m) {
    const f32x4 bias = ld4(tabqkv + m * 16 + 4 * g);
#pragma unroll
    for (int w = 0; w < 3; ++w) QKV[m][w] = bias;
  }
  gemm3<3 * G::TP, G::KQ_D, G::KS_D, G::MT_D>(QKV, A, X, lane);
}

template <int H, int NM>
PGP_DEV void qkv_fold(f32x4 (&acc)[NM][3], int T0, int n, const float* tab, const float (&ba)[3], int lane, int g) {
  using G = Geo<H>;
#pragma unroll
  for (int m = 0; m < NM; ++m)
    if (m < n) {
      const float a = tab[G::T_F0 + (T0 + m) * 64 + lane];
#pragma unroll
      for (int w = 0; w < 3; ++w)
        acc[m][w] = mfma(a, ba[w], ld4(tab + G::T_F0B + (w * 3 * G::NQT + T0 + m) * 16 + 4 * g));
    }
}
template <int H>
PGP_DEV float row_fold_part(int m, int n, int w, const float* tab, const float (&ba)[3], int g) {
  using G = Geo<H>;
  const float t = tab[G::T_F0R + (m * G::SR + n) * 4 + g];
  return (g < 3 ? t : 0.f) * ba[w];
}
template <int H>
PGP_DEV float row_fold_bias(int m, int n, int w, const float* tab) {
  using G = Geo<H>;
  return tab[G::T_F0RB + w * 3 * G::SR + m * G::SR + n];
}

template <int H, bool F0, bool SPLIT>
PGP_DEV void encoder_layer_tail(f32x4 (&X)[Geo<H>::MT_D][3], Ring<H, SPLIT>& ring, const float* TL, int lane,
                                const float* tab, const float (&ba)[3], const float (&xv)[3][3]) {
  using G = Geo<H>;
  constexpr int TQ = G::TQ, SR = G::SR, HF = G::HF;
  const int g = lane >> 4;
  constexpr bool BIL = F0;
  f32x4 QK[BIL ? 1 : 2 * TQ][3];
  float qr[SR][3], kr[SR][3];
  if constexpr (BIL) {
  } else {
#pragma unroll
    for (int m = 0; m < 2 * TQ; ++m) {
      const f32x4 bias = ld4(TL + G::TL_QKV + m * 16 + 4 * g);
#pragma unroll
      for (int w = 0; w < 3; ++w) QK[m][w] = bias;
    }
    float qkr[2 * SR][3];
    zero_rows(qkr);
    gemm3_rows<2 * TQ, G::KQ_D, G::KS_D, G::MT_D, 2 * TQ, 2 * SR>(QK, ring.cur, X, lane, qkr, TL + G::TL_RQ, g);
    rows_finish(qkr);
#pragma unroll
    for (int n = 0; n < SR; ++n)
#pragma unroll
      for (int w = 0; w < 3; ++w) {
        qr[n][w] = qkr[n][w] + TL[G::TL_RQB + n];
        kr[n][w] = qkr[SR + n][w] + TL[G::TL_RQB + SR + n];
      }
  }
  ring.advance();
  float P0[3][3], P1[3][3];
  if constexpr (BIL) {
#pragma unroll
    for (int hh = 0; hh < 2; ++hh) {
      const float* SB = tab + G::T_F0S + hh * 36;
      float tk[3][3], vk[3][3];
#pragma unroll
      for (int w2 = 0; w2 < 3; ++w2) {
#pragma unroll
        for (int f = 0; f < 3; ++f)
          tk[w2][f] = fmaf(SB[3 * f + 2], xv[w2][2], fmaf(SB[3 * f + 1], xv[w2][1], fmaf(SB[3 * f], xv[w2][0], SB[9 + 3 * f + w2])));
#pragma unroll
        for (int w = 0; w < 3; ++w)
          vk[w][w2] = fmaf(SB[18 + 3 * w + 2], xv[w2][2], fmaf(SB[18 + 3 * w + 1], xv[w2][1], fmaf(SB[18 + 3 * w], xv[w2][0], SB[27 + 3 * w + w2])));
      }
#pragma unroll
      for (int w = 0; w < 3; ++w) {
        float s[3];
#pragma unroll
        for (int w2 = 0; w2 < 3; ++w2)
          s[w2] = fmaf(xv[w][2], tk[w2][2], fmaf(xv[w][1], tk[w2][1], fmaf(xv[w][0], tk[w2][0], vk[w][w2])));
        const float m = fmaxf(s[0], fmaxf(s[1], s[2]));
        const float e0 = __expf(s[0] - m), e1 = __expf(s[1] - m), e2 = __expf(s[2] - m);
        const float iv = __builtin_amdgcn_rcpf(e0 + e1 + e2);
        float(&Pw)[3][3] = hh == 0 ? P0 : P1;
        Pw[w][0] = e0 * iv;
        Pw[w][1] = e1 * iv;
        Pw[w][2] = e2 * iv;
      }
    }
  } else
#pragma unroll
  for (int w = 0; w < 3; ++w) {
    float s0[3], s1[3];
#pragma unroll
    for (int w2 = 0; w2 < 3; ++w2) {
      float a0 = 0.f, a1 = 0.f;
#pragma unroll
      for (int t = 0; t < HF; ++t)
#pragma unroll
        for (int r = 0; r < 4; ++r) {
          a0 = fmaf(QK[t][w][r], QK[TQ + t][w2][r], a0);
          a1 = fmaf(QK[HF + t][w][r], QK[TQ + HF + t][w2][r], a1);
        }
#pragma unroll
      for (int r = 0; r < 4; ++r) {
        const float pr = QK[2 * HF][w][r] * QK[TQ + 2 * HF][w2][r];
        if (4 * r + g < G::HT)
          a0 += pr;
        else
          a1 += pr;
      }
      xsum2(a0, a1);
      s0[w2] = a0;
      float t1 = a1;
#pragma unroll
      for (int n = 0; n < SR; ++n) t1 = fmaf(qr[n][w], kr[n][w2], t1);
      s1[w2] = t1;
    }
    const float m0 = fmaxf(s0[0], fmaxf(s0[1], s0[2])), m1 = fmaxf(s1[0], fmaxf(s1[1], s1[2]));
    const float e00 = __expf(s0[0] - m0), e01 = __expf(s0[1] - m0), e02 = __expf(s0[2] - m0);
    const float e10 = __expf(s1[0] - m1), e11 = __expf(s1[1] - m1), e12 = __expf(s1[2] - m1);
    const float i0 = __builtin_amdgcn_rcpf(e00 + e01 + e02), i1 = __builtin_amdgcn_rcpf(e10 + e11 + e12);
    P0[w][0] = e00 * i0;
    P0[w][1] = e01 * i0;
    P0[w][2] = e02 * i0;
    P1[w][0] = e10 * i1;
    P1[w][1] = e11 * i1;
    P1[w][2] = e12 * i1;
  }
  f32x4 acc[G::MT_D][3];
#pragma unroll
  for (int mt = 0; mt < G::MT_D; ++mt) {
    const f32x4 bo = ld4(TL + G::TL_BO + 16 * mt + 4 * g);
    if constexpr (F0) {
#pragma unroll
      for (int w = 0; w < 3; ++w) acc[mt][w] = bo + X[mt][w];
    } else {
      const f32x4 g0 = ld4(TL - G::TL_SIZE + G::TL_LN2G + 16 * mt + 4 * g);
#pragma unroll
      for (int w = 0; w < 3; ++w) acc[mt][w] = X[mt][w] * g0 + bo;
    }
  }
  if constexpr (F0) {
#pragma unroll
    for (int w = 0; w < 3; ++w) {
      const float y0 = P0[w][0] * ba[0] + P0[w][1] * ba[1] + P0[w][2] * ba[2];
      const float y1 = P1[w][0] * ba[0] + P1[w][1] * ba[1] + P1[w][2] * ba[2];
      const float p0 = g == 0 ? P0[w][0] : g == 1 ? P0[w][1] : g == 2 ? P0[w][2] : 0.f;
      const float p1 = g == 0 ? P1[w][0] : g == 1 ? P1[w][1] : g == 2 ? P1[w][2] : 0.f;
      const float bops[4] = {y0, p0, y1, p1};
#pragma unroll
      for (int k = 0; k < 4; ++k)
#pragma unroll
        for (int mt = 0; mt < G::MT_X; ++mt)
          acc[mt][w] = mfma(tab[G::T_F0O + (k * G::MT_X + mt) * 64 + lane], bops[k], acc[mt][w]);
      float ro[G::XR];
#pragma unroll
      for (int n = 0; n < G::XR; ++n) {
        const float* rw = tab + G::T_F0OR + n * 16;
        ro[n] = g < 3 ? rw[g] * y0 + rw[4 + g] * p0 + rw[8 + g] * y1 + rw[12 + g] * p1 : 0.f;
      }
      acc[G::MT_X][w][0] += xsum_rows<G::XR>(ro);
    }
    layer_norm_tiles<H, false>(acc, X, TL + G::TL_LN1G, TL + G::TL_LN1B, g);
  } else {
  f32x4 V[TQ][3];
  float vr[SR][3];
#pragma unroll
  for (int t = 0; t < TQ; ++t) {
    const f32x4 bias = ld4(TL + G::TL_QKV + (2 * TQ + t) * 16 + 4 * g);
#pragma unroll
    for (int w = 0; w < 3; ++w) V[t][w] = bias;
  }
  zero_rows(vr);
  gemm3_rows<TQ, G::KQ_D, G::KS_D, G::MT_D, TQ, SR>(V, ring.cur, X, lane, vr, TL + G::TL_RQ + 2 * SR * G::KQ_D * 16,
                                                         g);
  float vd[3];
  {
    const float vb = TL[G::TL_RQB + 2 * SR + g];
#pragma unroll
    for (int w = 0; w < 3; ++w) vd[w] = rows_pick<SR>(vr, w) + (g < SR ? vb : 0.f);
  }
  f32x4 O[TQ + 1][3];
#pragma unroll
  for (int w = 0; w < 3; ++w) {
#pragma unroll
    for (int t = 0; t < 2 * HF; ++t) {
      const float(&Pw)[3][3] = t < HF ? P0 : P1;
      O[t][w] = Pw[w][0] * V[t][0] + Pw[w][1] * V[t][1] + Pw[w][2] * V[t][2];
    }
#pragma unroll
    for (int r = 0; r < 4; ++r) {
      const bool h0 = 4 * r + g < G::HT;
      const float c0 = h0 ? P0[w][0] : P1[w][0], c1 = h0 ? P0[w][1] : P1[w][1], c2 = h0 ? P0[w][2] : P1[w][2];
      O[2 * HF][w][r] = c0 * V[2 * HF][0][r] + c1 * V[2 * HF][1][r] + c2 * V[2 * HF][2][r];
    }
    const float o3 = P1[w][0] * vd[0] + P1[w][1] * vd[1] + P1[w][2] * vd[2];
    O[TQ][w] = f32x4{o3, 0.f, 0.f, 0.f};
  }
  {
    float ro[G::XR][3];
    zero_rows(ro);
    gemm3_rows<G::MT_X, G::KQ_OT, G::KS_OT, TQ + 1, G::MT_D, G::XR>(acc, ring.cur + G::G_V * G::FQ, O, lane, ro,
                                                                   TL + G::TL_RO, g);
#pragma unroll
    for (int w = 0; w < 3; ++w) acc[G::MT_X][w][0] += rows_pick<G::XR>(ro, w);
  }
  layer_norm_tiles<H, false>(acc, X, TL + G::TL_LN1G, TL + G::TL_LN1B, g);
  }
  ring.advance();
#pragma unroll
  for (int mt = 0; mt < G::MT_D; ++mt) {
    const f32x4 b2 = ld4(TL + G::TL_B2 + 16 * mt + 4 * g), g1 = ld4(TL + G::TL_LN1G + 16 * mt + 4 * g);
#pragma unroll
    for (int w = 0; w < 3; ++w) acc[mt][w] = X[mt][w] * g1 + b2;
  }
  if constexpr (SPLIT) {
    using S = EncS<H>;
    static_assert(S::NBF * 2 == G::MT_F, "hidden pairs");
    const float* A1 = ring.cur;
    const float* A2 = ring.cur + S::F1S * G::FQ;
#pragma unroll
    for (int w = 0; w < 3; ++w) {
      f32x4 F[G::MT_F];
#pragma unroll
      for (int c = 0; c < G::MT_F; ++c) F[c] = ld4(TL + G::TL_B1 + 16 * c + 4 * g);
      if constexpr (kEncPipe) {
        constexpr int QN = S::NBD * G::MT_F;
        u32x4 wn[3];
        planes_lds(A1, lane, wn);
#pragma unroll
        for (int b = 0; b < S::NBD; ++b) {
          u32x4 xb[3];
          {
            float v[8];
            pair_tiles<G::MT_D>(X, b, w, v);
            split8(v, xb);
          }
          prio_mfma();
#pragma unroll
          for (int c = 0; c < G::MT_F; ++c) {
            u32x4 wp[3];
#pragma unroll
            for (int k = 0; k < 3; ++k) wp[k] = wn[k];
            const int q = b * G::MT_F + c + 1;
            if (q < QN) planes_lds(A1 + (((q % G::MT_F) * S::NBD + q / G::MT_F) * 3) * 256, lane, wn);
            __builtin_amdgcn_sched_barrier(0);
            F[c] = mfma_bf6(wp, xb, F[c]);
          }
          prio_valu();
        }
      } else {
        u32x4 xs[S::NBD][3];
#pragma unroll
        for (int b = 0; b < S::NBD; ++b) {
          float v[8];
          pair_tiles<G::MT_D>(X, b, w, v);
          split8(v, xs[b]);
        }
        prio_mfma();
#pragma unroll
        for (int b = 0; b < S::NBD; ++b)
#pragma unroll
          for (int c = 0; c < G::MT_F; ++c) {
            u32x4 wp[3];
            planes_lds(A1 + ((c * S::NBD + b) * 3) * 256, lane, wp);
            F[c] = mfma_bf6(wp, xs[b], F[c]);
          }
        prio_valu();
      }
#pragma unroll
      for (int c = 0; c < G::MT_F; ++c)
#pragma unroll
        for (int r = 0; r < 4; ++r) F[c][r] = relu_enc<H>(F[c][r]);
      float rf[G::XR];
#pragma unroll
      for (int n = 0; n < G::XR; ++n) rf[n] = 0.f;
#pragma unroll
      for (int c = 0; c < G::MT_F; ++c)
#pragma unroll
        for (int n = 0; n < G::XR; ++n) {
          const f32x4 rw = ld4(TL + G::TL_RF + ((n * G::KQ_F + c) * 4 + g) * 4);
#pragma unroll
          for (int e = 0; e < 4; ++e) rf[n] = fmaf(rw[e], F[c][e], rf[n]);
        }
      if constexpr (kEncPipe) {
        constexpr int QN = S::NBF * G::MT_X;
        u32x4 wn[3];
        planes_lds(A2, lane, wn);
#pragma unroll
        for (int b = 0; b < S::NBF; ++b) {
          u32x4 hb[3];
          {
            float v[8];
#pragma unroll
            for (int e = 0; e < 4; ++e) {
              v[e] = F[2 * b][e];
              v[4 + e] = F[2 * b + 1][e];
            }
            split8(v, hb);
          }
          prio_mfma();
#pragma unroll
          for (int m = 0; m < G::MT_X; ++m) {
            u32x4 wp[3];
#pragma unroll
            for (int k = 0; k < 3; ++k) wp[k] = wn[k];
            const int q = b * G::MT_X + m + 1;
            if (q < QN) planes_lds(A2 + (((q % G::MT_X) * S::NBF + q / G::MT_X) * 3) * 256, lane, wn);
            __builtin_amdgcn_sched_barrier(0);
            acc[m][w] = mfma_bf6(wp, hb, acc[m][w]);
          }
          prio_valu();
        }
      } else {
        u32x4 hs[S::NBF][3];
#pragma unroll
        for (int b = 0; b < S::NBF; ++b) {
          float v[8];
#pragma unroll
          for (int e = 0; e < 4; ++e) {
            v[e] = F[2 * b][e];
            v[4 + e] = F[2 * b + 1][e];
          }
          split8(v, hs[b]);
        }
        prio_mfma();
#pragma unroll
        for (int b = 0; b < S::NBF; ++b)
#pragma unroll
          for (int m = 0; m < G::MT_X; ++m) {
            u32x4 wp[3];
            planes_lds(A2 + ((m * S::NBF + b) * 3) * 256, lane, wp);
            acc[m][w] = mfma_bf6(wp, hs[b], acc[m][w]);
          }
        prio_valu();
      }
      acc[G::MT_X][w][0] += xsum_rows<G::XR>(rf);
    }
  } else {
    static_assert(G::KQ_F == G::MT_F, "hidden tile c = W2 k-group c");
    float rf[G::XR][3];
    zero_rows(rf);
#pragma unroll
    for (int c = 0; c < G::MT_F; ++c) {
      f32x4 Fc[1][3];
      const f32x4 b1 = ld4(TL + G::TL_B1 + 16 * c + 4 * g);
#pragma unroll
      for (int w = 0; w < 3; ++w) Fc[0][w] = b1;
      gemm3<1, G::KQ_D, G::KS_D, G::MT_D>(Fc, ring.cur + c * G::KQ_D * 256, X, lane);
#pragma unroll
      for (int w = 0; w < 3; ++w)
#pragma unroll
        for (int r = 0; r < 4; ++r) Fc[0][w][r] = relu_enc<H>(Fc[0][w][r]);
      const float* A2 = ring.cur + G::G_F1 * G::FQ;
      prio_mfma();
#pragma unroll
      for (int m = 0; m < G::MT_X; ++m) {
        const f32x4 a = ld4(A2 + (m * G::KQ_F + c) * 256 + lane * 4);
#pragma unroll
        for (int e = 0; e < 4; ++e)
#pragma unroll
          for (int w = 0; w < 3; ++w) acc[m][w] = mfma(a[e], Fc[0][w][e], acc[m][w]);
      }
      prio_valu();
#pragma unroll
      for (int n = 0; n < G::XR; ++n) {
        const f32x4 rw = ld4(TL + G::TL_RF + ((n * G::KQ_F + c) * 4 + g) * 4);
#pragma unroll
        for (int e = 0; e < 4; ++e)
#pragma unroll
          for (int w = 0; w < 3; ++w) rf[n][w] = fmaf(rw[e], Fc[0][w][e], rf[n][w]);
      }
    }
#pragma unroll
    for (int w = 0; w < 3; ++w) acc[G::MT_X][w][0] += rows_pick<G::XR>(rf, w);
  }
  ring.advance();
  layer_norm_tiles<H, false>(acc, X, TL + G::TL_LN2G, TL + G::TL_LN2B, g);
}

template <int H, bool F0>
PGP_DEV void encoder_layer(f32x4 (&X)[Geo<H>::MT_D][3], Ring<H>& ring, const float* TL, int lane,
                           const float* tab, const float (&ba)[3]) {
  using G = Geo<H>;
  const int g = lane >> 4;
  f32x4 acc[G::MT_D][3];
  f32x4 QKV[3 * G::TP][3];
  f32x4 O[G::TP][3];
  if constexpr (F0)
    qkv_fold<H, 3 * G::TP>(QKV, 0, 3 * G::TP, tab, ba, lane, g);
  else
    qkv_gemm<H>(QKV, ring.cur, TL + G::TL_QKV, X, lane, g);
  ring.advance();
  attention<H>(QKV, O);
#pragma unroll
  for (int mt = 0; mt < G::MT_D; ++mt) {
    const f32x4 bo = ld4(TL + G::TL_BO + 16 * mt + 4 * g);
    if constexpr (F0) {
#pragma unroll
      for (int w = 0; w < 3; ++w) acc[mt][w] = bo + X[mt][w];
    } else {
      const f32x4 g0 = ld4(TL - G::TL_SIZE + G::TL_LN2G + 16 * mt + 4 * g);
#pragma unroll
      for (int w = 0; w < 3; ++w) acc[mt][w] = X[mt][w] * g0 + bo;
    }
  }
  gemm3<G::MT_D, G::KQ_O, G::KS_O, G::TP>(acc, ring.cur, O, lane);
  if constexpr (G::NPASS == 2) {
    if constexpr (F0)
      qkv_fold<H, 3 * G::TP>(QKV, 3 * G::TP, 3 * G::TP, tab, ba, lane, g);
    else
      qkv_gemm<H>(QKV, ring.cur + G::G_O * G::FQ, TL + G::TL_QKV + 3 * G::TP * 16, X, lane, g);
    ring.advance();
    attention<H>(QKV, O);
    gemm3<G::MT_D, G::KQ_O, G::KS_O, G::TP>(acc, ring.cur, O, lane);
  }
  layer_norm_tiles<H, false>(acc, X, TL + G::TL_LN1G, TL + G::TL_LN1B, g);
  f32x4 F1[G::MT_F][3];
#pragma unroll
  for (int mt = 0; mt < G::MT_F; ++mt) {
    const f32x4 b1 = ld4(TL + G::TL_B1 + 16 * mt + 4 * g);
#pragma unroll
    for (int w = 0; w < 3; ++w) F1[mt][w] = b1;
  }
  gemm3<G::MT_F, G::KQ_D, G::KS_D, G::MT_D>(F1, ring.cur + G::G_O * G::FQ, X, lane);
#pragma unroll
  for (int mt = 0; mt < G::MT_F; ++mt)
#pragma unroll
    for (int w = 0; w < 3; ++w)
#pragma unroll
      for (int r = 0; r < 4; ++r) F1[mt][w][r] = relu_enc<H>(F1[mt][w][r]);
  ring.advance();
#pragma unroll
  for (int mt = 0; mt < G::MT_D; ++mt) {
    const f32x4 b2 = ld4(TL + G::TL_B2 + 16 * mt + 4 * g), g1 = ld4(TL + G::TL_LN1G + 16 * mt + 4 * g);
#pragma unroll
    for (int w = 0; w < 3; ++w) acc[mt][w] = X[mt][w] * g1 + b2;
  }
  gemm3<G::MT_D, G::KQ_F, 16, G::MT_F>(acc, ring.cur, F1, lane);
  ring.advance();
  layer_norm_tiles<H, false>(acc, X, TL + G::TL_LN2G, TL + G::TL_LN2B, g);
}

template <int H, bool SPLIT>
__global__ __launch_bounds__(enc_waves<H>() * 64, H <= 16 ? kEnc16EU : tail_res<H>() ? 1 : 2) void encoder_kernel(
    FwdArgs a) {
  using G = Geo<H>;
  using L = EncLds<H, SPLIT>;
  __shared__ __attribute__((aligned(16))) float smem[L::TOTAL];
  __shared__ float xstage[L::UNITS ? NW_STAGE<H>() * 144 : 1];
  float* tab = smem + (L::RESIDENT ? L::STREAM : 2 * L::SLOT);
  const int tsz = G::t_size(a.K);
  for (int i = threadIdx.x; i < tsz; i += blockDim.x) tab[i] = a.tab[i];

  const int lane = threadIdx.x & 63, g = lane >> 4, j = lane & 15;
  const int wv = __builtin_amdgcn_readfirstlane(threadIdx.x >> 6);
  constexpr int NW = enc_waves<H>();
  const long nblk = (a.B + 15) / 16;

  Ring<H, SPLIT> ring{smem, smem + L::SLOT, a.frags + G::OFF_ENC, 0, H * kLayers * G::NST, wv, lane};
  if constexpr (SPLIT) {
    dma_groups(a.encb, smem, EncS<H>::GROUPS, wv, NW, lane);
    ring.nxt = smem;
    ring.next = 1;
    __syncthreads();
  } else if constexpr (L::RESIDENT) {
    dma_groups(a.frags + G::OFF_ENC + (long)L::RES0 * G::FQ, smem, kLayers * G::LAYER_G - L::RES0, wv, NW, lane);
    ring.nxt = smem;
    ring.next = 1;
    __syncthreads();
  } else {
    ring.nxt = smem;
    ring.issue();
    ring.nxt = smem + L::SLOT;
    ring.next = 1;
    __syncthreads();
    ring.issue();
  }

  auto unit = [&](long blk, int h, bool active, const float* pre) {
    const float* agg = a.agg + (active ? blk : 0) * H * 3 * 48;
    float* lat = a.lat + (active ? blk : 0) * G::LAT_BLK;
    float ba[3];
    float xv[3][3];
    if constexpr (L::UNITS) {
#pragma unroll
      for (int w = 0; w < 3; ++w) {
#pragma unroll
        for (int f = 0; f < 3; ++f) xv[w][f] = G::TAIL ? pre[w * 48 + 16 * f + j] : 0.f;
        const float v = pre[w * 48 + (lane < 48 ? lane : 47)];
        ba[w] = g < 3 ? v : 0.f;
      }
    } else {
#pragma unroll
      for (int w = 0; w < 3; ++w) ba[w] = (active && g < 3) ? agg[(h * 3 + w) * 48 + lane] : 0.f;
#pragma unroll
      for (int w = 0; w < 3; ++w)
#pragma unroll
        for (int f = 0; f < 3; ++f)
          xv[w][f] = (G::TAIL && active) ? agg[(h * 3 + w) * 48 + 16 * f + j] : 0.f;
    }
    f32x4 X[G::MT_D][3];
#pragma unroll
    for (int mt = 0; mt < G::MT_D; ++mt) {
      const float aw = tab[G::T_TEW + mt * 64 + lane];
#pragma unroll
      for (int w = 0; w < 3; ++w) X[mt][w] = mfma(aw, ba[w], ld4(tab + G::T_TE + w * G::DP + 16 * mt + 4 * g));
    }
    static_assert(kLayers == 2, "layer 0 (folded q/k/v) + layer 1");
    if constexpr (G::TAIL) {
      encoder_layer_tail<H, true, SPLIT>(X, ring, tab + G::T_L0, lane, tab, ba, xv);
      encoder_layer_tail<H, false, SPLIT>(X, ring, tab + G::T_L0 + G::TL_SIZE, lane, tab, ba, xv);
    } else if constexpr (!SPLIT) {
      encoder_layer<H, true>(X, ring, tab + G::T_L0, lane, tab, ba);
      encoder_layer<H, false>(X, ring, tab + G::T_L0 + G::TL_SIZE, lane, tab, ba);
    }

    if (active) {
#pragma unroll
      for (int w = 0; w < 3; ++w) {
        float* lc = lat + (long)((h * 3 + w) * G::KS_D) * 64;
#pragma unroll
        for (int q = 0; q < G::LAT_FG; ++q) *reinterpret_cast<f32x4*>(lc + q * 256 + lane * 4) = X[q][w];
        if constexpr (G::KS_D % 4 != 0) {
#pragma unroll
          for (int r = 0; r < G::KS_D % 4; ++r) lc[G::LAT_FG * 256 + r * 64 + lane] = X[G::LAT_FG][w][r];
        }
      }
      if (a.latent != nullptr) {
        const long b = blk * 16 + j;
        if (b < a.B) {
#pragma unroll
          for (int w = 0; w < 3; ++w)
#pragma unroll
            for (int mt = 0; mt < G::MT_D; ++mt)
#pragma unroll
              for (int r = 0; r < 4; ++r) {
                const int c = 16 * mt + 4 * r + g;
                const float* TL1 = tab + G::T_L0 + G::TL_SIZE;
                if (c < H)
                  a.latent[b * G::LAT + (long)h * 3 * H + w * H + c] =
                      X[mt][w][r] * TL1[G::TL_LN2G + 16 * mt + 4 * g + r] + TL1[G::TL_LN2B + 16 * mt + 4 * g + r];
              }
        }
      }
    }
  };
  if constexpr (L::UNITS) {
    const long U = nblk * H, NWT = (long)gridDim.x * NW, gw = (long)blockIdx.x * NW + wv;
    const long u1 = (gw + 1) * U / NWT;
    float* slot = xstage + wv * 144;
    const long u0 = gw * U / NWT;
    float pf[3];
    auto load_x = [&](long u) {
#pragma unroll
      for (int k = 0; k < 3; ++k) pf[k] = a.agg[u * 144 + (64 * k + lane < 144 ? 64 * k + lane : 143)];
    };
    auto stage_x = [&]() {
#pragma unroll
      for (int k = 0; k < 3; ++k)
        if (64 * k + lane < 144) slot[64 * k + lane] = pf[k];
    };
    if (u0 < u1) {
      load_x(u0);
      stage_x();
    }
#pragma unroll 1
    for (long u = u0; u < u1; ++u) {
      load_x(u + 1 < u1 ? u + 1 : u);
      const long blk = u / H;
      unit(blk, (int)(u - blk * H), true, slot);
      stage_x();
    }
  } else {
    const long blk = (long)blockIdx.x * NW + wv;
    const bool active = blk < nblk;
#pragma unroll 1
    for (int h = 0; h < H; ++h) unit(blk, h, active, nullptr);
  }
}

template <int H, bool SPLIT>
hipError_t launch_form(const FwdArgs& a, hipStream_t st) {
  const long nblk = (a.B + 15) / 16;
  constexpr int NW = enc_waves<H>();
  long grid = (nblk + NW - 1) / NW;
  static std::atomic<int> fits{-1};
  if (fits.load(std::memory_order_relaxed) < 0) {
    hipFuncAttributes fa{};
    const bool ok = hipFuncGetAttributes(&fa, reinterpret_cast<const void*>(encoder_kernel<H, SPLIT>)) == hipSuccess &&
                    fa.maxThreadsPerBlock >= NW * 64;
    fits.store(ok ? 1 : 0, std::memory_order_relaxed);
  }
  if (!fits.load(std::memory_order_relaxed)) return hipErrorLaunchOutOfResources;
  if constexpr (EncLds<H>::UNITS) {
    static std::atomic<int> occ_cache{0};
    int occ = occ_cache.load(std::memory_order_relaxed);
    if (occ <= 0) {
      if (hipOccupancyMaxActiveBlocksPerMultiprocessor(&occ, encoder_kernel<H, SPLIT>, NW * 64, 0) != hipSuccess ||
          occ <= 0)
        occ = 1;
      occ_cache.store(occ, std::memory_order_relaxed);
    }
    grid = std::min<long>((long)device_cus() * occ, (nblk * H + NW - 1) / NW);
  }
  encoder_kernel<H, SPLIT><<<(int)grid, NW * 64, 0, st>>>(a);
  return hipGetLastError();
}

template <int H>
hipError_t launch(const FwdArgs& a, hipStream_t st) {
  if constexpr (enc_split<H>())
    if (a.encb != nullptr) return launch_form<H, true>(a, st);
  return launch_form<H, false>(a, st);
}

template <int H>
hipError_t launch_split(const float* frags, float* encb, hipStream_t st) {
  if constexpr (enc_split<H>()) {
    using G = Geo<H>;
    constexpr long n = 2L * (G::MT_F * EncS<H>::NBD + G::MT_X * EncS<H>::NBF) + G::P_F1;
    enc_split_kernel<H><<<(int)((n + 3) / 4), 256, 0, st>>>(frags + G::OFF_ENC, encb);
    return hipGetLastError();
  }
  return hipErrorInvalidValue;
}

}

hipError_t launch_encoder(const FwdArgs& a, hipStream_t st) {
  switch (a.H) {
#define CASE(h) \
  case h:       \
    return launch<h>(a, st);
    PGP_FOR_EACH_H(CASE)
#undef CASE
  }
  return hipErrorInvalidValue;
}

long encoder_split_floats(int H) {
  switch (H) {
#define CASE(h) \
  case h:       \
    return enc_split<h>() ? EncS<h>::SIZE : 0;
    PGP_FOR_EACH_H(CASE)
#undef CASE
  }
  return 0;
}

hipError_t launch_encoder_split(int H, const float* frags, float* encb, hipStream_t st) {
  switch (H) {
#define CASE(h) \
  case h:       \
    return launch_split<h>(frags, encb, st);
    PGP_FOR_EACH_H(CASE)
#undef CASE
  }
  return hipErrorInvalidValue;
}

}
```

### preganplus_amd/model.py

```python
from __future__ import annotations

import ctypes

import numpy as np
import torch

from . import _native
from . import weights as W


class DecisionModel:
    def __init__(self, n_hosts: int, weights: dict, device: str | torch.device = "cuda"):
        self.H = int(n_hosts)
        self.K = int(np.asarray(weights["prototypes"]).shape[0])
        self.device = torch.device(device)
        if self.device.type == "cuda" and self.device.index is None:
            self.device = torch.device("cuda", torch.cuda.current_device())
        if self.device.type != "cuda":
            raise ValueError("DecisionModel runs on the GPU only (no CPU fallback)")
        L = _native.lib()
        if self.H not in _native.supported_hosts():
            raise ValueError(f"H={self.H} not compiled in; supported {_native.supported_hosts()}")
        self._L = L
        h = ctypes.c_void_p()
        _native.check(L.pgp_create(self.H, self.K, ctypes.byref(h)), "pgp_create")
        self._h = h
        self.load_weights(weights)

    def load_weights(self, weights: dict):
        blob = W.pack_blob(weights, self.H)
        n = self._L.pgp_weight_blob_len(self.H, self.K)
        if n != blob.size:
            raise ValueError(f"blob length {blob.size} != {n}")
        torch.cuda.set_device(self.device)
        _native.check(self._L.pgp_load_weights(
            self._h, blob.ctypes.data_as(ctypes.POINTER(ctypes.c_double)), blob.size),
            "pgp_load_weights")
        self.prototypes = np.asarray(weights["prototypes"], dtype=np.float64)

    def load_master(self, P: torch.Tensor, prototypes):
        pr = np.ascontiguousarray(np.asarray(prototypes, dtype=np.float64))
        L = self._L
        L.pgp_load_weights_master.argtypes = [ctypes.c_void_p, ctypes.c_void_p, ctypes.POINTER(ctypes.c_double)]
        torch.cuda.synchronize(self.device)
        _native.check(L.pgp_load_weights_master(self._h, ctypes.c_void_p(P.data_ptr()),
                                                pr.ctypes.data_as(ctypes.POINTER(ctypes.c_double))),
                      "pgp_load_weights_master")
        self.prototypes = pr.copy()

    def repack_master(self, P: torch.Tensor, protos_dev: torch.Tensor, prototypes_host=None, stream=None,
                      sections: int = 3):
        if protos_dev.dtype != torch.float64 or protos_dev.numel() != 2 * self.K or not protos_dev.is_contiguous():
            raise ValueError(f"protos_dev must be contiguous float64 [{self.K},2] on the device")
        L = self._L
        L.pgp_repack_master_sections.argtypes = [ctypes.c_void_p] * 3 + [ctypes.c_int, ctypes.c_void_p]
        st = stream if stream is not None else torch.cuda.current_stream(self.device)
        _native.check(L.pgp_repack_master_sections(self._h, ctypes.c_void_p(P.data_ptr()),
                                                   ctypes.c_void_p(protos_dev.data_ptr()), int(sections),
                                                   ctypes.c_void_p(st.cuda_stream)), "pgp_repack_master_sections")
        if prototypes_host is not None:
            self.prototypes = np.array(prototypes_host, dtype=np.float64)

    def reserve(self, max_batch: int):
        _native.check(self._L.pgp_reserve(self._h, int(max_batch)), "pgp_reserve")

    def gan_split(self, on: bool):
        _native.check(self._L.pgp_gan_split(self._h, int(bool(on))), "pgp_gan_split")

    def encoder_split(self, on: bool):
        _native.check(self._L.pgp_encoder_split(self._h, int(bool(on))), "pgp_encoder_split")

    def decoder_split(self, on: bool):
        _native.check(self._L.pgp_decoder_split(self._h, int(bool(on))), "pgp_decoder_split")

    def alloc_outputs(self, B: int, latent: bool = False, packed: bool = False):
        dev, H = self.device, self.H
        f32, i32 = torch.float32, torch.int32
        spec = [("logits", f32, (B, H, 2)), ("protos", f32, (B, H, 2)), ("cls", i32, (B, H)), ("any", i32, (B,)),
                ("probs", f32, (B, 2)), ("keep", i32, (B,)), ("final_target", i32, (B, H)),
                ("gen_target", i32, (B, H))]
        if packed:
            n = sum(int(np.prod(s)) for _, _, s in spec)
            buf = torch.zeros(n, dtype=i32, device=dev)
            out, o = {}, 0
            for name, dt, shp in spec:
                k = int(np.prod(shp))
                out[name] = buf[o:o + k].view(dt).view(shp)
                o += k
            out["_buf"] = buf
            out["_hbuf"] = torch.zeros(n, dtype=i32).pin_memory()
        else:
            out = {name: torch.empty(shp, dtype=dt, device=dev) for name, dt, shp in spec}
        out["latent"] = torch.empty((B, 3 * H * H), dtype=f32, device=dev) if latent else None
        return out

    def _check_inputs(self, windows, sched):
        H = self.H
        B = windows.shape[0]
        if tuple(windows.shape) != (B, 3, 3 * H) or windows.dtype != torch.float32:
            raise ValueError(f"windows must be float32 [B,3,{3 * H}], got {tuple(windows.shape)} {windows.dtype}")
        if sched is not None and (tuple(sched.shape) != (B, H, H) or sched.dtype != torch.float32):
            raise ValueError(f"sched must be float32 [B,{H},{H}], got {tuple(sched.shape)} {sched.dtype}")
        for t in (windows, sched):
            if t is not None and (t.device != self.device or not t.is_contiguous()):
                raise ValueError("inputs must be contiguous tensors on the model's device")
        return B

    def forward(self, windows: torch.Tensor, sched: torch.Tensor, out: dict | None = None,
                latent: bool = False, stage: int = -1, stream=None) -> dict:
        B = self._check_inputs(windows, sched)
        if out is None:
            out = self.alloc_outputs(B, latent)
        st = stream if stream is not None else torch.cuda.current_stream(self.device)
        p = lambda t: None if t is None else t.data_ptr()
        _native.check(self._L.pgp_forward_stage(
            self._h, int(stage), B, p(windows), p(sched), p(out["logits"]), p(out["protos"]),
            p(out["cls"]), p(out["any"]), p(out["probs"]), p(out["keep"]),
            p(out["final_target"]), p(out["gen_target"]), p(out.get("latent")),
            ctypes.c_void_p(st.cuda_stream)), "pgp_forward")
        return out

    def close(self):
        if getattr(self, "_h", None) is not None and self._h.value:
            self._L.pgp_destroy(self._h)
            self._h = None

    def __del__(self):
        try:
            self.close()
        except Exception:
            pass


class FPEDecisionModel(DecisionModel):

    def __init__(self, n_hosts: int, weights: dict, device: str | torch.device = "cuda"):
        self.H = int(n_hosts)
        self.K = W.FPE_PROTOS
        self.device = torch.device(device)
        if self.device.type == "cuda" and self.device.index is None:
            self.device = torch.device("cuda", torch.cuda.current_device())
        if self.device.type != "cuda":
            raise ValueError("FPEDecisionModel runs on the GPU only (no CPU fallback)")
        L = _native.lib()
        self._L = L
        h = ctypes.c_void_p()
        _native.check(L.pgp_create_fpe(self.H, ctypes.byref(h)), "pgp_create_fpe")
        self._h = h
        self.load_weights(weights)

    def load_weights(self, weights: dict):
        if "fpe" not in weights:
            raise ValueError("FPE weights need an 'fpe' section (PreGAN FPE_16 state_dict)")
        blob = W.pack_blob(weights, self.H)
        n = self._L.pgp_fpe_weight_blob_len(self.H)
        if n != blob.size:
            raise ValueError(f"blob length {blob.size} != {n}")
        torch.cuda.set_device(self.device)
        _native.check(self._L.pgp_load_weights(
            self._h, blob.ctypes.data_as(ctypes.POINTER(ctypes.c_double)), blob.size), "pgp_load_weights")
        self.prototypes = np.asarray(weights["prototypes"], dtype=np.float64)

    def load_master(self, P, prototypes):
        raise NotImplementedError("the PreGAN encoder is frozen (PreGAN.py:29); reload GAN weights with load_weights")

    def alloc_outputs(self, B: int, latent: bool = False):
        out = super().alloc_outputs(B, False)
        out["scores"] = out.pop("logits")
        return out

    def forward(self, windows: torch.Tensor, h0: torch.Tensor, sched: torch.Tensor, out: dict | None = None,
                stage: int = -1, stream=None) -> dict:
        B = self._check_inputs(windows, sched)
        if tuple(h0.shape) != (B, 3) or h0.dtype != torch.float32 or h0.device != self.device \
                or not h0.is_contiguous():
            raise ValueError(f"h0 must be contiguous float32 [B,3] on {self.device}")
        if out is None:
            out = self.alloc_outputs(B)
        st = stream if stream is not None else torch.cuda.current_stream(self.device)
        p = lambda t: t.data_ptr()
        _native.check(self._L.pgp_forward_fpe_stage(
            self._h, int(stage), B, p(windows), p(h0), p(sched), p(out["scores"]), p(out["protos"]), p(out["cls"]),
            p(out["any"]), p(out["probs"]), p(out["keep"]), p(out["final_target"]), p(out["gen_target"]),
            ctypes.c_void_p(st.cuda_stream)), "pgp_forward_fpe")
        return out


def migrations(keep_orig: torch.Tensor, final_target: torch.Tensor, cur_host: torch.Tensor, stream=None,
               out=None):
    B, C = final_target.shape
    for t, shp in ((keep_orig, (B,)), (final_target, (B, C)), (cur_host, (B, C))):
        if tuple(t.shape) != shp or t.dtype != torch.int32 or not t.is_cuda or not t.is_contiguous():
            raise ValueError("migrations: int32 contiguous device tensors keep [B], final_target/cur_host [B,C]")
    moves, hosts_from = out if out is not None else (torch.empty_like(final_target), torch.empty_like(final_target))
    st = stream if stream is not None else torch.cuda.current_stream(final_target.device)
    _native.check(_native.lib().pgp_migrations(
        C, B, keep_orig.data_ptr(), final_target.data_ptr(), cur_host.data_ptr(), moves.data_ptr(),
        hosts_from.data_ptr(), ctypes.c_void_p(st.cuda_stream)), "pgp_migrations")
    return moves, hosts_from


def embedding(logits: torch.Tensor, protos: torch.Tensor, out: torch.Tensor | None = None, stream=None):
    B, H = logits.shape[0], logits.shape[1]
    for t in (logits, protos):
        if tuple(t.shape) != (B, H, 2) or t.dtype != torch.float32 or not t.is_cuda or not t.is_contiguous():
            raise ValueError("embedding: fp32 contiguous device tensors logits / protos [B,H,2]")
    out = torch.empty_like(protos) if out is None else out
    st = stream if stream is not None else torch.cuda.current_stream(logits.device)
    _native.check(_native.lib().pgp_embedding(H, B, logits.data_ptr(), protos.data_ptr(), out.data_ptr(),
                                              ctypes.c_void_p(st.cuda_stream)), "pgp_embedding")
    return out


def assemble_decision(original_decision, moves_row, cur_host_row):
    decision = dict(original_decision)
    moves_row = [int(v) for v in moves_row]
    cur = [int(v) for v in cur_host_row]
    order = sorted((h, c) for c, h in enumerate(cur) if h >= 0)
    for _, c in order:
        if moves_row[c] >= 0:
            decision[c] = moves_row[c]
    return list(decision.items())


def to_numpy(out: dict) -> dict:
    res = {}
    if "_buf" in out:
        hb = out["_hbuf"]
        hb.copy_(out["_buf"], non_blocking=True)
        torch.cuda.current_stream(out["_buf"].device).synchronize()
        a, o = hb.numpy(), 0
        for k, v in out.items():
            if k.startswith("_") or v is None or k == "latent":
                continue
            n = v.numel()
            x = a[o:o + n].view(np.float32 if v.dtype == torch.float32 else np.int32).reshape(tuple(v.shape)).copy()
            res[k] = x.astype(bool) if k in ("any", "keep") else x
            o += n
        if out.get("latent") is not None:
            res["latent"] = out["latent"].detach().cpu().numpy()
        return res
    for k, v in out.items():
        if v is None or k.startswith("_"):
            continue
        a = v.detach().cpu().numpy()
        if k in ("any", "keep"):
            a = a.astype(bool)
        res[k] = a
    return res
```

### preganplus_amd/roofline.py

```python
from __future__ import annotations

PEAK_FP32_TFLOPS = 157.3
PEAK_HBM_GBS = 8000.0
PEAK_BF16_TFLOPS = 2500.0

W = 3
FF = 64
GAN_HIDDEN = 64


def macs_per_window(H: int) -> dict:
    d = H
    tokens = W * H
    hd = d // 2
    gat = tokens * 3 * d + 2 * tokens * d + W * H * H * d
    te = tokens * d * d
    per_token_layer = 3 * d * d + d * d + 2 * (W * hd) * 2 + 2 * FF * d
    layers = 2 * tokens * per_token_layer
    dec = (W * H * d) * (4 * H)
    gan = GAN_HIDDEN * (2 * H + H * H) + (H * H) * GAN_HIDDEN + GAN_HIDDEN * 2 * H * H + 2 * GAN_HIDDEN
    return dict(gat=gat, time_encoder=te, encoder_layers=layers, decoders=dec, gan=gan)


def flops_per_window(H: int) -> dict:
    return {k: 2 * v for k, v in macs_per_window(H).items()}


def total_flops_per_window(H: int) -> int:
    return sum(flops_per_window(H).values())


def encdec_flops_per_window(H: int) -> int:
    f = flops_per_window(H)
    return f["time_encoder"] + f["encoder_layers"] + f["decoders"]


def encoder_flops_per_window(H: int) -> int:
    f = flops_per_window(H)
    return f["time_encoder"] + f["encoder_layers"]


ENC_MFMA_PER_HOST = {16: 264, 50: 1116}


def encoder_executed_flops_per_window(H: int):
    n = ENC_MFMA_PER_HOST.get(H)
    return None if n is None else n * 2048 * H / 16


ENC_SPLIT_MFMA_PER_HOST = {50: (516, 504)}


def encoder_split(H: int) -> bool:
    return H in ENC_SPLIT_MFMA_PER_HOST


def encoder_split_executed_flops_per_window(H: int):
    f32, bf = ENC_SPLIT_MFMA_PER_HOST[H]
    return f32 * 2048 * H / 16, bf * 16 * 16 * 32 * 2 * H / 16


TUNE_MFMA_PER_UNIT = {
    16: {"tf_fwd_kernel": 156, "tf_bwd_ffn_kernel": 288, "tf_bwd_att_kernel": 96},
    50: {"tf_fwd_kernel": 840, "tf_bwd_ffn_kernel": 384, "tf_bwd_att_kernel": 1200},
}
TUNE_BF16_PER_UNIT = {
    16: {"tf_fwd_kernel": 0, "tf_bwd_ffn_kernel": 0, "tf_bwd_att_kernel": 0},
    50: {"tf_fwd_kernel": 288, "tf_bwd_ffn_kernel": 576, "tf_bwd_att_kernel": 144},
}
TUNE_FUSED_LAUNCHES = ("fwd layer 0", "fwd layer 1", "ffn bwd layer 1", "att bwd layer 1", "ffn bwd layer 0",
                       "att bwd layer 0")


def tf_grid(units: int, waves: int, cus: int, reserve: int = 0) -> int:
    r = max(0, min(reserve, cus // 2))
    gmax = max(1, min(cus - r, (units + waves - 1) // waves))
    m = (units + waves * gmax - 1) // (waves * gmax)
    return max(1, (units + waves * m - 1) // (waves * m))


def tune_fused_grids(H: int, B: int, B_fwd: int | None, cus: int, reserve: int = 0):
    units = (B * H + 15) // 16
    ufwd = ((B if B_fwd is None else B_fwd) * H + 15) // 16
    gf, gb = tf_grid(ufwd, 8, cus, reserve), tf_grid(units, 4, cus, reserve)
    return [gf, gf, gb, gb, gb, gb]


def tune_te_mfma(H: int) -> int:
    nt = (H + 15) // 16
    ks = 4 * (H // 16) + (min(H % 16, 4) if H % 16 else 0)
    return nt * ks * 3


def tune_fused_flops(H: int, B: int, B_fwd: int | None = None):
    c = TUNE_MFMA_PER_UNIT.get(H)
    if c is None:
        return None
    bf = TUNE_BF16_PER_UNIT.get(H, {})
    eq = {k: n * 2048 + bf.get(k, 0) * 16 * 16 * 32 * 2 * PEAK_FP32_TFLOPS / PEAK_BF16_TFLOPS for k, n in c.items()}
    units = (B * H + 15) // 16
    ufwd = ((B if B_fwd is None else B_fwd) * H + 15) // 16
    fwd, te = eq["tf_fwd_kernel"], tune_te_mfma(H) * 2048
    return ([ufwd * fwd, ufwd * (fwd - te)]
            + [units * n for n in (eq["tf_bwd_ffn_kernel"], eq["tf_bwd_att_kernel"], eq["tf_bwd_ffn_kernel"],
                                   eq["tf_bwd_att_kernel"])])


def encoder_io_bytes_per_window(H: int) -> int:
    return 4 * (W * H * 3) + 4 * (W * H * H)


def decoder_flops_per_window(H: int) -> int:
    return flops_per_window(H)["decoders"]


def decoder_split(H: int) -> bool:
    return H in (32, 50)


def gan_split(H: int) -> bool:
    return H in (16, 50)


def gan_split_flops_per_window(H: int, onehot: bool = True) -> int:
    ep = (2 * H + 15) // 16
    npe = (ep + 1) // 2
    nps = ((H * H + 15) // 16 + 1) // 2
    mtn = (H + 15) // 16
    npn = (mtn + 1) // 2
    n = npe * 4 * 6 + nps * 8 * (3 if onehot else 6) + H * (mtn * 2 * 6 + 4 * npn * 6)
    return n * 16 * 16 * 32 * 2 // 16


def decoder_split_flops_per_window(H: int) -> int:
    ks = (H + 3) // 4
    nb = ((ks + 3) // 4 + 1) // 2
    mt = (4 * H + 15) // 16
    return H * W * nb * mt * 6 * 16 * 16 * 32 * 2 // 16


def gan_flops_per_window(H: int) -> int:
    return flops_per_window(H)["gan"]


def path_bytes_per_window(H: int) -> int:
    return 36 * H + 4 * H * H + 8 * H + 8 * H + 4 * H + 4 * H + 8


def fpe_macs_per_window(H: int = 16) -> int:
    E, L = H + 3, 10
    gru = W * (9 * 3 * H + 9 * 3)
    gat = W * (H * 3 * H + 2 * H * H + H * H * H)
    mha = W * 3 * E * E + 2 * W * W * E + W * E * E
    enc = W * E * L * H
    dec = H * (2 * L + 2 * L)
    return gru + gat + mha + enc + dec


def fpe_flops_per_window(H: int = 16) -> int:
    return 2 * fpe_macs_per_window(H)


def fpe_executed_flops_per_window(H: int = 16) -> int:
    per_step = H * (27 + 6) * 2 + 27 * 2 + H * H * (2 + 4) + H * (3 + 3 + 2) * 2
    mha = 3 * (36 + 6) * 2 + 9 * 6 * 2 + 3 * 3 * 6 * 2
    out = 4 * H * 18 * 2
    return 3 * per_step + mha + out


def fpe_bytes_per_window(H: int = 16) -> int:
    return 36 * H + 12 + 8 * H + 8 * H + 4 * H + 4 + 8 * H


def tune_step_flops_per_window(H: int) -> int:
    f = flops_per_window(H)
    return 3 * (f["gat"] + f["time_encoder"] + f["encoder_layers"] + f["decoders"])


def gan_step_macs_per_env(H: int, hidden: int = GAN_HIDDEN) -> int:
    gin, hh = 2 * H + H * H, H * H
    fwd = hidden * gin + hh * hidden + hidden * 2 * hh + 2 * hidden
    disc_step = 2 * hidden + 2 * hidden + hidden * 2 * hh
    gen_step = hidden * 2 * hh + 2 * hidden + 2 * hidden + 3 * hh * hidden + hidden * gin
    return fwd + disc_step + gen_step


def gan_step_flops_per_env(H: int) -> int:
    return 2 * gan_step_macs_per_env(H)
```

Baseline: 647.2 million host-windows/s.

## Add attention-split bf16 encoder form with LDS-resident pre-split weight triples

Adds a third encoder form that pre-splits the attention Q/K/V and output-projection weights into bf16 triples, alongside the existing split feed-forward weights. It makes this form the default when the split buffer exists. The Q/K/V and output GEMMs run as bf16x3 MFMA with software-pipelined plane loads, reading mostly from LDS with one streamed triple from global memory. The goal is to replace fp32 MFMA in attention with cheaper split-bf16 MFMA. In exchange it uses more LDS, which may lower occupancy, and adds register pressure and extra split-weight preparation.

```diff
diff --git a/include/preganplus.h b/include/preganplus.h
--- a/include/preganplus.h
+++ b/include/preganplus.h
@@ -46,6 +46,7 @@
 int pgp_embedding(int n_hosts, int batch, const float* logits, const float* protos, float* emb, void* stream);
 int pgp_decoder_split(pgp_model* m, int on);
 int pgp_encoder_split(pgp_model* m, int on);
+int pgp_encoder_form_info(int n_hosts, int* compiled, int* lds_bytes, int* resident_triples, int* streamed_triples);
 int pgp_gan_split(pgp_model* m, int on);
 int pgp_schedule_onehot(int n_hosts, int batch, const unsigned char* idx, float* sched, void* stream);
 
diff --git a/preganplus_amd/_native.py b/preganplus_amd/_native.py
--- a/preganplus_amd/_native.py
+++ b/preganplus_amd/_native.py
@@ -76,6 +76,9 @@
     L.pgp_decoder_split.restype = c_int
     L.pgp_encoder_split.argtypes = [vp, c_int]
     L.pgp_encoder_split.restype = c_int
+    if hasattr(L, "pgp_encoder_form_info"):
+        L.pgp_encoder_form_info.argtypes = [c_int] + [ctypes.POINTER(c_int)] * 4
+        L.pgp_encoder_form_info.restype = c_int
     L.pgp_gan_split.argtypes = [vp, c_int]
     L.pgp_gan_split.restype = c_int
     L.pgp_schedule_onehot.argtypes = [c_int, c_int, fp, fp, vp]
diff --git a/preganplus_amd/csrc/pgp_capi.hip b/preganplus_amd/csrc/pgp_capi.hip
--- a/preganplus_amd/csrc/pgp_capi.hip
+++ b/preganplus_amd/csrc/pgp_capi.hip
@@ -11,6 +11,10 @@
 #include "pgp_tunef.hpp"
 #include "pgp_tunedp.hpp"
 
+#ifndef PGP_ENC_FORM
+#define PGP_ENC_FORM 1
+#endif
+
 #include <vector>
 
 using namespace pgp;
@@ -22,7 +26,7 @@
   float* d_frags = nullptr;
   float* d_decb = nullptr;
   float* d_encb = nullptr;
-  bool enc_split = true;
+  int enc_form = PGP_ENC_FORM;
   bool dec_split = true;
   float* d_ganb = nullptr;
   bool gan_split = true;
@@ -216,7 +220,8 @@
   a.emb = m->d_emb;
   a.frags = m->d_frags;
   a.decb = m->dec_split ? m->d_decb : nullptr;
-  a.encb = m->enc_split ? m->d_encb : nullptr;
+  a.encb = m->enc_form ? m->d_encb : nullptr;
+  a.enc_form = m->enc_form;
   a.ganb = m->gan_split ? m->d_ganb : nullptr;
   a.tab = m->d_tab;
   a.gtab = m->d_gtab;
@@ -329,7 +334,15 @@
   if (!m) return fail(PGP_ERR_ARG, "NULL model");
   if (m->fpe || encoder_split_floats(m->H) == 0)
     return on ? fail(PGP_ERR_UNSUPPORTED, "split-bf16 encoder not compiled for this model / host count") : PGP_OK;
-  m->enc_split = on != 0;
+  if (on < 0 || on > 2) return fail(PGP_ERR_ARG, "encoder form: 0 (fp32), 1 (best split form) or 2 (split feed-forward)");
+  m->enc_form = on;
+  return PGP_OK;
+}
+
+int pgp_encoder_form_info(int n_hosts, int* compiled, int* lds_bytes, int* resident_triples, int* streamed_triples) {
+  if (!compiled || !lds_bytes || !resident_triples || !streamed_triples) return fail(PGP_ERR_ARG, "NULL output");
+  *compiled = encoder_asplit(n_hosts) ? 1 : 0;
+  encoder_asplit_geometry(n_hosts, lds_bytes, resident_triples, streamed_triples);
   return PGP_OK;
 }
 
diff --git a/preganplus_amd/csrc/pgp_device.hpp b/preganplus_amd/csrc/pgp_device.hpp
--- a/preganplus_amd/csrc/pgp_device.hpp
+++ b/preganplus_amd/csrc/pgp_device.hpp
@@ -29,6 +29,7 @@
 
 struct FwdArgs {
   int B, H, K;
+  int enc_form;
   const float* windows;
   const float* sched;
   float* agg;
@@ -99,6 +100,8 @@
 hipError_t launch_decoder_split(int H, const float* frags, float* decb, hipStream_t st);
 long encoder_split_floats(int H);
 hipError_t launch_encoder_split(int H, const float* frags, float* encb, hipStream_t st);
+bool encoder_asplit(int H);
+void encoder_asplit_geometry(int H, int* lds_bytes, int* resident, int* streamed);
 hipError_t launch_gan(const FwdArgs& a, hipStream_t st);
 long gan_split_floats(int H);
 hipError_t launch_gan_split_derive(int H, const float* frags, float* planes, hipStream_t st);
diff --git a/preganplus_amd/csrc/pgp_encoder.hip b/preganplus_amd/csrc/pgp_encoder.hip
--- a/preganplus_amd/csrc/pgp_encoder.hip
+++ b/preganplus_amd/csrc/pgp_encoder.hip
@@ -38,11 +38,29 @@
   static constexpr long SIZE = STREAM;
 };
 
-template <int H, bool SPLIT = false>
+template <int H>
+struct EncA {
+  using G = Geo<H>;
+  using S = EncS<H>;
+  static constexpr int NBD = S::NBD;
+  static constexpr int NBO = cdiv(G::KQ_OT, 2);
+  static constexpr int TQK = 2 * G::TQ * NBD, TV = G::TQ * NBD, TO = G::MT_X * NBO;
+  static constexpr int NT = TQK + TV + TO;
+  static constexpr int NRES = TQK + TV - 1;
+  static constexpr int L0F = 0, L1F = S::FFN, L1A = 2 * S::FFN;
+  static constexpr int RES_G = L1A + 3 * NRES;
+  static constexpr int GROUPS = L1A + 3 * NT;
+  static constexpr long SIZE = (long)GROUPS * G::FQ;
+};
+
+template <int H, bool SPLIT = false, bool AS = false>
 struct EncLds {
+  static_assert(SPLIT || !AS, "the attention-split form includes the split feed-forward");
   static constexpr bool TRES = tail_res<H>();
   static constexpr int RES0 = TRES ? Geo<H>::st_begin(Geo<H>::NST - 1) : 0;
-  static constexpr int STREAM = SPLIT ? EncS<H>::STREAM : (kLayers * Geo<H>::LAYER_G - RES0) * Geo<H>::FQ;
+  static constexpr int STREAM = AS      ? EncA<H>::RES_G * Geo<H>::FQ
+                                : SPLIT ? EncS<H>::STREAM
+                                        : (kLayers * Geo<H>::LAYER_G - RES0) * Geo<H>::FQ;
   static constexpr bool RESIDENT = TRES || STREAM * 4 <= 32 * 1024;
   static constexpr int SLOT = Geo<H>::SLOT_G * Geo<H>::FQ;
   static constexpr int TAB = Geo<H>::t_size(kMaxProtos);
@@ -53,6 +71,81 @@
 template <int H>
 constexpr bool enc_split() {
   return tail_res<H>() && EncLds<H, true>::TOTAL * 4 + enc_waves<H>() * 144 * 4 <= 160 * 1024;
+}
+
+template <int H>
+constexpr int enc_asplit_lds_bytes() {
+  return EncLds<H, true, true>::TOTAL * 4 + enc_waves<H>() * 144 * 4;
+}
+template <int H>
+constexpr bool enc_asplit() {
+  return enc_split<H>() && enc_asplit_lds_bytes<H>() <= 160 * 1024;
+}
+
+PGP_DEV void split_groups(const float* src, long q0, long q1, float* dst, int lane) {
+  float v[8];
+  const f32x4 x0 = ld4(src + q0 * 256 + lane * 4);
+  const f32x4 x1 = q1 >= 0 ? ld4(src + q1 * 256 + lane * 4) : f32x4{0.f, 0.f, 0.f, 0.f};
+#pragma unroll
+  for (int e = 0; e < 4; ++e) {
+    v[e] = x0[e];
+    v[4 + e] = x1[e];
+  }
+  u32x4 p[3];
+  split8(v, p);
+#pragma unroll
+  for (int k = 0; k < 3; ++k) *reinterpret_cast<u32x4*>(dst + k * 256 + lane * 4) = p[k];
+}
+
+template <int H>
+__global__ __launch_bounds__(256) void enc_asplit_kernel(const float* __restrict__ enc, float* __restrict__ out) {
+  using G = Geo<H>;
+  using S = EncS<H>;
+  using A = EncA<H>;
+  constexpr int T1 = G::MT_F * S::NBD, T2 = G::MT_X * S::NBF, TL = T1 + T2;
+  const long f = (long)blockIdx.x * 4 + (threadIdx.x >> 6);
+  const int lane = threadIdx.x & 63;
+  if (f >= 2 * TL + A::NT) return;
+  const float* src;
+  long q0, q1, dst;
+  if (f < 2 * TL) {
+    const int l = (int)(f / TL), t = (int)(f % TL);
+    src = enc + (long)(l * G::LAYER_G + G::P_F1) * 256;
+    const long base = l == 0 ? A::L0F : A::L1F;
+    if (t < T1) {
+      const int c = t / S::NBD, b = t % S::NBD;
+      q0 = c * G::KQ_D + 2 * b;
+      q1 = 2 * b + 1 < G::KQ_D ? q0 + 1 : -1;
+      dst = base + (long)t * 3;
+    } else {
+      const int u = t - T1, m = u / S::NBF, b = u % S::NBF;
+      q0 = G::G_F1 + m * G::KQ_F + 2 * b;
+      q1 = q0 + 1;
+      dst = base + S::F1S + (long)u * 3;
+    }
+  } else {
+    const int t = (int)(f - 2 * TL);
+    src = enc + (long)G::LAYER_G * 256;
+    int b, kq;
+    if (t < A::TQK) {
+      b = t / (2 * G::TQ);
+      kq = G::KQ_D;
+      q0 = (t % (2 * G::TQ)) * G::KQ_D + 2 * b;
+    } else if (t < A::TQK + A::TV) {
+      const int u = t - A::TQK;
+      b = u / G::TQ;
+      kq = G::KQ_D;
+      q0 = G::P_V + (u % G::TQ) * G::KQ_D + 2 * b;
+    } else {
+      const int u = t - A::TQK - A::TV;
+      b = u / G::MT_X;
+      kq = G::KQ_OT;
+      q0 = G::P_OT + (u % G::MT_X) * G::KQ_OT + 2 * b;
+    }
+    q1 = 2 * b + 1 < kq ? q0 + 1 : -1;
+    dst = A::L1A + (long)t * 3;
+  }
+  split_groups(src, q0, q1, out + dst * 256, lane);
 }
 
 template <int H>
@@ -121,6 +214,114 @@
 PGP_DEV void prio_mfma() { __builtin_amdgcn_s_setprio(1); }
 PGP_DEV void prio_valu() { __builtin_amdgcn_s_setprio(0); }
 
+template <int H>
+PGP_DEV void att_planes(const float* AL, const float* __restrict__ AG, int t, int lane, u32x4 (&w)[3]) {
+  unsigned off = (unsigned)lane * 16u;
+  asm volatile("" : "+v"(off));
+  if (t < EncA<H>::NRES) {
+#pragma unroll
+    for (int k = 0; k < 3; ++k)
+      w[k] = *reinterpret_cast<const u32x4*>(reinterpret_cast<const char*>(AL + (t * 3 + k) * 256) + off);
+  } else {
+#pragma unroll
+    for (int k = 0; k < 3; ++k)
+      w[k] = *reinterpret_cast<const u32x4*>(reinterpret_cast<const char*>(AG + (t * 3 + k) * 256) + off);
+  }
+}
+template <int H, int T0, int NTR, int D>
+PGP_DEV void att_prologue(const float* AL, const float* AG, int lane, u32x4 (&wq)[NTR][3]) {
+  __builtin_amdgcn_sched_barrier(0);
+#pragma unroll
+  for (int t = 0; t < D && t < NTR; ++t) att_planes<H>(AL, AG, T0 + t, lane, wq[t]);
+  __builtin_amdgcn_sched_barrier(0);
+}
+template <int KQ, int KS, int NB, int NR>
+PGP_DEV void att_rows(float (&racc)[NR][3], const float* RW, const f32x4 (&Bx)[NB][3], int b, int w, int g) {
+#pragma unroll
+  for (int q4 = 2 * b; q4 < 2 * b + 2 && q4 < KQ; ++q4) {
+    unsigned goff = (unsigned)g * 16u;
+    asm volatile("" : "+v"(goff));
+    f32x4 rw[NR];
+#pragma unroll
+    for (int n = 0; n < NR; ++n)
+      rw[n] = *reinterpret_cast<const f32x4*>(reinterpret_cast<const char*>(RW + (n * KQ + q4) * 16) + goff);
+#pragma unroll
+    for (int e = 0; e < 4; ++e)
+      if (4 * q4 + e < KS) {
+#pragma unroll
+        for (int n = 0; n < NR; ++n) racc[n][w] = fmaf(rw[n][e], Bx[q4][w][e], racc[n][w]);
+      }
+  }
+}
+template <int H, int T0, int NM, int KQ, int KS, int NB, int NMA, int NR, int TH = -1>
+PGP_DEV void att_gemm_steps(f32x4 (&acc)[NMA][3], const float* AL, const float* AG, const f32x4 (&Bx)[NB][3], int lane,
+                            float (&racc)[NR][3], const float* RW, int g, const u32x4 (&wh)[3]) {
+  static_assert(NM <= NMA, "accumulator tiles");
+  constexpr int NBK = cdiv(KQ, 2), NTR = NM * NBK;
+  u32x4 wn[3];
+  att_planes<H>(AL, AG, T0, lane, wn);
+#pragma unroll
+  for (int w = 0; w < 3; ++w) {
+#pragma unroll
+    for (int b = 0; b < NBK; ++b) {
+      u32x4 xb[3];
+      {
+        float v[8];
+        pair_tiles<NB>(Bx, b, w, v);
+        split8(v, xb);
+      }
+      prio_mfma();
+#pragma unroll
+      for (int m = 0; m < NM; ++m) {
+        u32x4 wp[3];
+#pragma unroll
+        for (int k = 0; k < 3; ++k) wp[k] = wn[k];
+        const int q = (b * NM + m + 1) % NTR;
+        if (T0 + q == TH) {
+#pragma unroll
+          for (int k = 0; k < 3; ++k) wn[k] = wh[k];
+        } else if (q != 0 || w < 2) {
+          att_planes<H>(AL, AG, T0 + q, lane, wn);
+        }
+        __builtin_amdgcn_sched_barrier(0);
+        acc[m][w] = mfma_bf6(wp, xb, acc[m][w]);
+        if (m == 0) att_rows<KQ, KS, NB, NR>(racc, RW, Bx, b, w, g);
+      }
+      prio_valu();
+    }
+  }
+}
+
+template <int H, int T0, int NM, int KQ, int KS, int NB, int NMA, int NR, int D>
+PGP_DEV void att_gemm(f32x4 (&acc)[NMA][3], u32x4 (&wq)[NM * cdiv(KQ, 2)][3], const float* AL, const float* AG,
+                      const f32x4 (&Bx)[NB][3], int lane, float (&racc)[NR][3], const float* RW, int g) {
+  static_assert(NM <= NMA, "accumulator tiles");
+  constexpr int NBK = cdiv(KQ, 2), NTR = NM * NBK;
+#pragma unroll
+  for (int b = 0; b < NBK; ++b) {
+    u32x4 xb[3][3];
+#pragma unroll
+    for (int w = 0; w < 3; ++w) {
+      float v[8];
+      pair_tiles<NB>(Bx, b, w, v);
+      split8(v, xb[w]);
+    }
+    prio_mfma();
+#pragma unroll
+    for (int m = 0; m < NM; ++m) {
+      const int t = b * NM + m;
+      if (t + D < NTR) att_planes<H>(AL, AG, T0 + t + D, lane, wq[t + D]);
+      __builtin_amdgcn_sched_barrier(0);
+#pragma unroll
+      for (int w = 0; w < 3; ++w) {
+        acc[m][w] = mfma_bf6(wq[t], xb[w], acc[m][w]);
+        if (m == 0) att_rows<KQ, KS, NB, NR>(racc, RW, Bx, b, w, g);
+      }
+    }
+    prio_valu();
+  }
+}
+
 template <int NM, int KQ, int KS, int NB, int NMA = NM>
 PGP_DEV void gemm3(f32x4 (&acc)[NMA][3], const float* A, const f32x4 (&Bx)[NB][3], int lane) {
   static_assert(NM <= NMA, "accumulator tiles");
@@ -242,10 +443,10 @@
   }
 }
 
-template <int H, bool SPLIT = false>
+template <int H, bool SPLIT = false, bool AS = false>
 struct Ring {
   using G = Geo<H>;
-  static constexpr bool RES = EncLds<H, SPLIT>::RESIDENT;
+  static constexpr bool RES = EncLds<H, SPLIT, AS>::RESIDENT;
   float* cur;
   float* nxt;
   const float* enc;
@@ -264,7 +465,9 @@
     if constexpr (RES) {
       const int si = next % (kLayers * G::NST), l = si / G::NST, k = si % G::NST;
       int gi;
-      if constexpr (SPLIT)
+      if constexpr (AS)
+        gi = l == 0 ? EncA<H>::L0F : k == 2 ? EncA<H>::L1F : EncA<H>::L1A;
+      else if constexpr (SPLIT)
         gi = l == 0 ? EncS<H>::L0F : k == 2 ? EncS<H>::L1F : EncS<H>::L1A + G::st_begin(k);
       else
         gi = l * G::LAYER_G + G::st_begin(k) - EncLds<H>::RES0;
@@ -360,12 +563,16 @@
   return tab[G::T_F0RB + w * 3 * G::SR + m * G::SR + n];
 }
 
-template <int H, bool F0, bool SPLIT>
-PGP_DEV void encoder_layer_tail(f32x4 (&X)[Geo<H>::MT_D][3], Ring<H, SPLIT>& ring, const float* TL, int lane,
+template <int H, bool F0, bool SPLIT, bool AS = false>
+PGP_DEV void encoder_layer_tail(f32x4 (&X)[Geo<H>::MT_D][3], Ring<H, SPLIT, AS>& ring, const float* TL, int lane,
                                 const float* tab, const float (&ba)[3], const float (&xv)[3][3]) {
   using G = Geo<H>;
   constexpr int TQ = G::TQ, SR = G::SR, HF = G::HF;
   const int g = lane >> 4;
+  using EA = EncA<H>;
+  constexpr int kAhead = 1;
+  const float* AL = ring.nxt + EA::L1A * G::FQ;
+  const float* AG = ring.enc + EA::L1A * G::FQ;
   constexpr bool BIL = F0;
   f32x4 QK[BIL ? 1 : 2 * TQ][3];
   float qr[SR][3], kr[SR][3];
@@ -379,7 +586,14 @@
     }
     float qkr[2 * SR][3];
     zero_rows(qkr);
-    gemm3_rows<2 * TQ, G::KQ_D, G::KS_D, G::MT_D, 2 * TQ, 2 * SR>(QK, ring.cur, X, lane, qkr, TL + G::TL_RQ, g);
+    if constexpr (AS) {
+      static_assert(EA::TQK <= EA::NRES, "q|k triples in LDS");
+      const u32x4 none[3] = {};
+      att_gemm_steps<H, 0, 2 * TQ, G::KQ_D, G::KS_D, G::MT_D, 2 * TQ, 2 * SR>(QK, AL, AG, X, lane, qkr,
+                                                                            TL + G::TL_RQ, g, none);
+    } else {
+      gemm3_rows<2 * TQ, G::KQ_D, G::KS_D, G::MT_D, 2 * TQ, 2 * SR>(QK, ring.cur, X, lane, qkr, TL + G::TL_RQ, g);
+    }
     rows_finish(qkr);
 #pragma unroll
     for (int n = 0; n < SR; ++n)
@@ -390,6 +604,12 @@
       }
   }
   ring.advance();
+  u32x4 vh[3] = {};
+  if constexpr (AS && !F0) {
+    static_assert(EA::NRES == EA::TQK + EA::TV - 1, "one v triple in the global image");
+    att_planes<H>(AL, AG, EA::NRES, lane, vh);
+    __builtin_amdgcn_sched_barrier(0);
+  }
   float P0[3][3], P1[3][3];
   if constexpr (BIL) {
 #pragma unroll
@@ -461,6 +681,7 @@
     P1[w][2] = e12 * i1;
   }
   f32x4 acc[G::MT_D][3];
+  if constexpr (F0 || !AS) {
 #pragma unroll
   for (int mt = 0; mt < G::MT_D; ++mt) {
     const f32x4 bo = ld4(TL + G::TL_BO + 16 * mt + 4 * g);
@@ -472,6 +693,7 @@
 #pragma unroll
       for (int w = 0; w < 3; ++w) acc[mt][w] = X[mt][w] * g0 + bo;
     }
+  }
   }
   if constexpr (F0) {
 #pragma unroll
@@ -505,8 +727,24 @@
     for (int w = 0; w < 3; ++w) V[t][w] = bias;
   }
   zero_rows(vr);
-  gemm3_rows<TQ, G::KQ_D, G::KS_D, G::MT_D, TQ, SR>(V, ring.cur, X, lane, vr, TL + G::TL_RQ + 2 * SR * G::KQ_D * 16,
-                                                         g);
+  if constexpr (AS) {
+    att_gemm_steps<H, EA::TQK, TQ, G::KQ_D, G::KS_D, G::MT_D, TQ, SR, EA::NRES>(
+        V, AL, AG, X, lane, vr, TL + G::TL_RQ + 2 * SR * G::KQ_D * 16, g, vh);
+  } else {
+    gemm3_rows<TQ, G::KQ_D, G::KS_D, G::MT_D, TQ, SR>(V, ring.cur, X, lane, vr, TL + G::TL_RQ + 2 * SR * G::KQ_D * 16,
+                                                      g);
+  }
+  u32x4 wo[AS ? EA::TO : 1][3];
+  if constexpr (AS) {
+    att_prologue<H, EA::TQK + EA::TV, EA::TO, kAhead>(AL, AG, lane, wo);
+#pragma unroll
+    for (int mt = 0; mt < G::MT_D; ++mt) {
+      const f32x4 bo = ld4(TL + G::TL_BO + 16 * mt + 4 * g);
+      const f32x4 g0 = ld4(TL - G::TL_SIZE + G::TL_LN2G + 16 * mt + 4 * g);
+#pragma unroll
+      for (int w = 0; w < 3; ++w) acc[mt][w] = X[mt][w] * g0 + bo;
+    }
+  }
   float vd[3];
   {
     const float vb = TL[G::TL_RQB + 2 * SR + g];
@@ -533,8 +771,12 @@
   {
     float ro[G::XR][3];
     zero_rows(ro);
-    gemm3_rows<G::MT_X, G::KQ_OT, G::KS_OT, TQ + 1, G::MT_D, G::XR>(acc, ring.cur + G::G_V * G::FQ, O, lane, ro,
-                                                                   TL + G::TL_RO, g);
+    if constexpr (AS)
+      att_gemm<H, EA::TQK + EA::TV, G::MT_X, G::KQ_OT, G::KS_OT, TQ + 1, G::MT_D, G::XR, kAhead>(
+          acc, wo, AL, AG, O, lane, ro, TL + G::TL_RO, g);
+    else
+      gemm3_rows<G::MT_X, G::KQ_OT, G::KS_OT, TQ + 1, G::MT_D, G::XR>(acc, ring.cur + G::G_V * G::FQ, O, lane, ro,
+                                                                     TL + G::TL_RO, g);
 #pragma unroll
     for (int w = 0; w < 3; ++w) acc[G::MT_X][w][0] += rows_pick<G::XR>(ro, w);
   }
@@ -778,150 +1020,41 @@
 template <int H, bool SPLIT>
 __global__ __launch_bounds__(enc_waves<H>() * 64, H <= 16 ? kEnc16EU : tail_res<H>() ? 1 : 2) void encoder_kernel(
     FwdArgs a) {
-  using G = Geo<H>;
+  constexpr bool AS = false;
   using L = EncLds<H, SPLIT>;
   __shared__ __attribute__((aligned(16))) float smem[L::TOTAL];
   __shared__ float xstage[L::UNITS ? NW_STAGE<H>() * 144 : 1];
-  float* tab = smem + (L::RESIDENT ? L::STREAM : 2 * L::SLOT);
-  const int tsz = G::t_size(a.K);
-  for (int i = threadIdx.x; i < tsz; i += blockDim.x) tab[i] = a.tab[i];
-
-  const int lane = threadIdx.x & 63, g = lane >> 4, j = lane & 15;
-  const int wv = __builtin_amdgcn_readfirstlane(threadIdx.x >> 6);
-  constexpr int NW = enc_waves<H>();
-  const long nblk = (a.B + 15) / 16;
-
-  Ring<H, SPLIT> ring{smem, smem + L::SLOT, a.frags + G::OFF_ENC, 0, H * kLayers * G::NST, wv, lane};
-  if constexpr (SPLIT) {
-    dma_groups(a.encb, smem, EncS<H>::GROUPS, wv, NW, lane);
-    ring.nxt = smem;
-    ring.next = 1;
-    __syncthreads();
-  } else if constexpr (L::RESIDENT) {
-    dma_groups(a.frags + G::OFF_ENC + (long)L::RES0 * G::FQ, smem, kLayers * G::LAYER_G - L::RES0, wv, NW, lane);
-    ring.nxt = smem;
-    ring.next = 1;
-    __syncthreads();
-  } else {
-    ring.nxt = smem;
-    ring.issue();
-    ring.nxt = smem + L::SLOT;
-    ring.next = 1;
-    __syncthreads();
-    ring.issue();
-  }
-
-  auto unit = [&](long blk, int h, bool active, const float* pre) {
-    const float* agg = a.agg + (active ? blk : 0) * H * 3 * 48;
-    float* lat = a.lat + (active ? blk : 0) * G::LAT_BLK;
-    float ba[3];
-    float xv[3][3];
-    if constexpr (L::UNITS) {
-#pragma unroll
-      for (int w = 0; w < 3; ++w) {
-#pragma unroll
-        for (int f = 0; f < 3; ++f) xv[w][f] = G::TAIL ? pre[w * 48 + 16 * f + j] : 0.f;
-        const float v = pre[w * 48 + (lane < 48 ? lane : 47)];
-        ba[w] = g < 3 ? v : 0.f;
-      }
-    } else {
-#pragma unroll
-      for (int w = 0; w < 3; ++w) ba[w] = (active && g < 3) ? agg[(h * 3 + w) * 48 + lane] : 0.f;
-#pragma unroll
-      for (int w = 0; w < 3; ++w)
-#pragma unroll
-        for (int f = 0; f < 3; ++f)
-          xv[w][f] = (G::TAIL && active) ? agg[(h * 3 + w) * 48 + 16 * f + j] : 0.f;
-    }
-    f32x4 X[G::MT_D][3];
-#pragma unroll
-    for (int mt = 0; mt < G::MT_D; ++mt) {
-      const float aw = tab[G::T_TEW + mt * 64 + lane];
-#pragma unroll
-      for (int w = 0; w < 3; ++w) X[mt][w] = mfma(aw, ba[w], ld4(tab + G::T_TE + w * G::DP + 16 * mt + 4 * g));
-    }
-    static_assert(kLayers == 2, "layer 0 (folded q/k/v) + layer 1");
-    if constexpr (G::TAIL) {
-      encoder_layer_tail<H, true, SPLIT>(X, ring, tab + G::T_L0, lane, tab, ba, xv);
-      encoder_layer_tail<H, false, SPLIT>(X, ring, tab + G::T_L0 + G::TL_SIZE, lane, tab, ba, xv);
-    } else if constexpr (!SPLIT) {
-      encoder_layer<H, true>(X, ring, tab + G::T_L0, lane, tab, ba);
-      encoder_layer<H, false>(X, ring, tab + G::T_L0 + G::TL_SIZE, lane, tab, ba);
-    }
-
-    if (active) {
-#pragma unroll
-      for (int w = 0; w < 3; ++w) {
-        float* lc = lat + (long)((h * 3 + w) * G::KS_D) * 64;
-#pragma unroll
-        for (int q = 0; q < G::LAT_FG; ++q) *reinterpret_cast<f32x4*>(lc + q * 256 + lane * 4) = X[q][w];
-        if constexpr (G::KS_D % 4 != 0) {
-#pragma unroll
-          for (int r = 0; r < G::KS_D % 4; ++r) lc[G::LAT_FG * 256 + r * 64 + lane] = X[G::LAT_FG][w][r];
-        }
-      }
-      if (a.latent != nullptr) {
-        const long b = blk * 16 + j;
-        if (b < a.B) {
-#pragma unroll
-          for (int w = 0; w < 3; ++w)
-#pragma unroll
-            for (int mt = 0; mt < G::MT_D; ++mt)
-#pragma unroll
-              for (int r = 0; r < 4; ++r) {
-                const int c = 16 * mt + 4 * r + g;
-                const float* TL1 = tab + G::T_L0 + G::TL_SIZE;
-                if (c < H)
-                  a.latent[b * G::LAT + (long)h * 3 * H + w * H + c] =
-                      X[mt][w][r] * TL1[G::TL_LN2G + 16 * mt + 4 * g + r] + TL1[G::TL_LN2B + 16 * mt + 4 * g + r];
-              }
-        }
-      }
-    }
-  };
-  if constexpr (L::UNITS) {
-    const long U = nblk * H, NWT = (long)gridDim.x * NW, gw = (long)blockIdx.x * NW + wv;
-    const long u1 = (gw + 1) * U / NWT;
-    float* slot = xstage + wv * 144;
-    const long u0 = gw * U / NWT;
-    float pf[3];
-    auto load_x = [&](long u) {
-#pragma unroll
-      for (int k = 0; k < 3; ++k) pf[k] = a.agg[u * 144 + (64 * k + lane < 144 ? 64 * k + lane : 143)];
-    };
-    auto stage_x = [&]() {
-#pragma unroll
-      for (int k = 0; k < 3; ++k)
-        if (64 * k + lane < 144) slot[64 * k + lane] = pf[k];
-    };
-    if (u0 < u1) {
-      load_x(u0);
-      stage_x();
-    }
-#pragma unroll 1
-    for (long u = u0; u < u1; ++u) {
-      load_x(u + 1 < u1 ? u + 1 : u);
-      const long blk = u / H;
-      unit(blk, (int)(u - blk * H), true, slot);
-      stage_x();
-    }
-  } else {
-    const long blk = (long)blockIdx.x * NW + wv;
-    const bool active = blk < nblk;
-#pragma unroll 1
-    for (int h = 0; h < H; ++h) unit(blk, h, active, nullptr);
-  }
-}
-
-template <int H, bool SPLIT>
+#include "pgp_encoder_body.inc"
+}
+
+template <int H>
+__global__ __launch_bounds__(enc_waves<H>() * 64, 1) void encoder_asplit_kernel(FwdArgs a) {
+  static_assert(enc_asplit<H>(), "LDS budget of the attention-split form");
+  constexpr bool SPLIT = true, AS = true;
+  using L = EncLds<H, true, true>;
+  __shared__ __attribute__((aligned(16))) float smem[L::TOTAL];
+  __shared__ float xstage[NW_STAGE<H>() * 144];
+#include "pgp_encoder_body.inc"
+}
+
+template <int H, bool SPLIT, bool AS>
+auto enc_kernel_ptr() {
+  if constexpr (AS)
+    return &encoder_asplit_kernel<H>;
+  else
+    return &encoder_kernel<H, SPLIT>;
+}
+
+template <int H, bool SPLIT, bool AS = false>
 hipError_t launch_form(const FwdArgs& a, hipStream_t st) {
+  const auto kern = enc_kernel_ptr<H, SPLIT, AS>();
   const long nblk = (a.B + 15) / 16;
   constexpr int NW = enc_waves<H>();
   long grid = (nblk + NW - 1) / NW;
   static std::atomic<int> fits{-1};
   if (fits.load(std::memory_order_relaxed) < 0) {
     hipFuncAttributes fa{};
-    const bool ok = hipFuncGetAttributes(&fa, reinterpret_cast<const void*>(encoder_kernel<H, SPLIT>)) == hipSuccess &&
+    const bool ok = hipFuncGetAttributes(&fa, reinterpret_cast<const void*>(kern)) == hipSuccess &&
                     fa.maxThreadsPerBlock >= NW * 64;
     fits.store(ok ? 1 : 0, std::memory_order_relaxed);
   }
@@ -930,19 +1063,20 @@
     static std::atomic<int> occ_cache{0};
     int occ = occ_cache.load(std::memory_order_relaxed);
     if (occ <= 0) {
-      if (hipOccupancyMaxActiveBlocksPerMultiprocessor(&occ, encoder_kernel<H, SPLIT>, NW * 64, 0) != hipSuccess ||
-          occ <= 0)
+      if (hipOccupancyMaxActiveBlocksPerMultiprocessor(&occ, kern, NW * 64, 0) != hipSuccess || occ <= 0)
         occ = 1;
       occ_cache.store(occ, std::memory_order_relaxed);
     }
     grid = std::min<long>((long)device_cus() * occ, (nblk * H + NW - 1) / NW);
   }
-  encoder_kernel<H, SPLIT><<<(int)grid, NW * 64, 0, st>>>(a);
+  kern<<<(int)grid, NW * 64, 0, st>>>(a);
   return hipGetLastError();
 }
 
 template <int H>
 hipError_t launch(const FwdArgs& a, hipStream_t st) {
+  if constexpr (enc_asplit<H>())
+    if (a.encb != nullptr && a.enc_form == 1) return launch_form<H, true, true>(a, st);
   if constexpr (enc_split<H>())
     if (a.encb != nullptr) return launch_form<H, true>(a, st);
   return launch_form<H, false>(a, st);
@@ -954,6 +1088,10 @@
     using G = Geo<H>;
     constexpr long n = 2L * (G::MT_F * EncS<H>::NBD + G::MT_X * EncS<H>::NBF) + G::P_F1;
     enc_split_kernel<H><<<(int)((n + 3) / 4), 256, 0, st>>>(frags + G::OFF_ENC, encb);
+    if constexpr (enc_asplit<H>()) {
+      constexpr long na = 2L * (G::MT_F * EncS<H>::NBD + G::MT_X * EncS<H>::NBF) + EncA<H>::NT;
+      enc_asplit_kernel<H><<<(int)((na + 3) / 4), 256, 0, st>>>(frags + G::OFF_ENC, encb + EncS<H>::SIZE);
+    }
     return hipGetLastError();
   }
   return hipErrorInvalidValue;
@@ -976,11 +1114,38 @@
   switch (H) {
 #define CASE(h) \
   case h:       \
-    return enc_split<h>() ? EncS<h>::SIZE : 0;
+    return enc_split<h>() ? EncS<h>::SIZE + (enc_asplit<h>() ? EncA<h>::SIZE : 0) : 0;
     PGP_FOR_EACH_H(CASE)
 #undef CASE
   }
   return 0;
+}
+
+bool encoder_asplit(int H) {
+  switch (H) {
+#define CASE(h) \
+  case h:       \
+    return enc_asplit<h>();
+    PGP_FOR_EACH_H(CASE)
+#undef CASE
+  }
+  return false;
+}
+
+void encoder_asplit_geometry(int H, int* lds_bytes, int* resident, int* streamed) {
+  *lds_bytes = *resident = *streamed = 0;
+  switch (H) {
+#define CASE(h)                                      \
+  case h:                                            \
+    if (enc_asplit<h>()) {                           \
+      *lds_bytes = enc_asplit_lds_bytes<h>();        \
+      *resident = EncA<h>::NRES;                     \
+      *streamed = EncA<h>::NT - EncA<h>::NRES;       \
+    }                                                \
+    return;
+    PGP_FOR_EACH_H(CASE)
+#undef CASE
+  }
 }
 
 hipError_t launch_encoder_split(int H, const float* frags, float* encb, hipStream_t st) {
diff --git a/preganplus_amd/csrc/pgp_encoder_body.inc b/preganplus_amd/csrc/pgp_encoder_body.inc
--- /dev/null
+++ b/preganplus_amd/csrc/pgp_encoder_body.inc
@@ -0,0 +1,138 @@
+  using G = Geo<H>;
+  float* tab = smem + (AS ? 0 : L::RESIDENT ? L::STREAM : 2 * L::SLOT);
+  const int tsz = G::t_size(a.K);
+  for (int i = threadIdx.x; i < tsz; i += blockDim.x) tab[i] = a.tab[i];
+
+  const int lane = threadIdx.x & 63, g = lane >> 4, j = lane & 15;
+  const int wv = __builtin_amdgcn_readfirstlane(threadIdx.x >> 6);
+  constexpr int NW = enc_waves<H>();
+  const long nblk = (a.B + 15) / 16;
+
+  Ring<H, SPLIT, AS> ring{smem, smem + L::SLOT, a.frags + G::OFF_ENC, 0, H * kLayers * G::NST, wv, lane};
+  if constexpr (AS) {
+    ring.enc = a.encb + EncS<H>::SIZE;
+    dma_groups(ring.enc, smem + L::TAB, EncA<H>::RES_G, wv, NW, lane);
+    ring.nxt = smem + L::TAB;
+    ring.next = 1;
+    __syncthreads();
+  } else if constexpr (SPLIT) {
+    dma_groups(a.encb, smem, EncS<H>::GROUPS, wv, NW, lane);
+    ring.nxt = smem;
+    ring.next = 1;
+    __syncthreads();
+  } else if constexpr (L::RESIDENT) {
+    dma_groups(a.frags + G::OFF_ENC + (long)L::RES0 * G::FQ, smem, kLayers * G::LAYER_G - L::RES0, wv, NW, lane);
+    ring.nxt = smem;
+    ring.next = 1;
+    __syncthreads();
+  } else {
+    ring.nxt = smem;
+    ring.issue();
+    ring.nxt = smem + L::SLOT;
+    ring.next = 1;
+    __syncthreads();
+    ring.issue();
+  }
+
+  auto unit = [&](long blk, int h, bool active, const float* pre) {
+    const float* agg = a.agg + (active ? blk : 0) * H * 3 * 48;
+    float* lat = a.lat + (active ? blk : 0) * G::LAT_BLK;
+    float ba[3];
+    float xv[3][3];
+    if constexpr (L::UNITS) {
+#pragma unroll
+      for (int w = 0; w < 3; ++w) {
+#pragma unroll
+        for (int f = 0; f < 3; ++f) xv[w][f] = G::TAIL ? pre[w * 48 + 16 * f + j] : 0.f;
+        const float v = pre[w * 48 + (lane < 48 ? lane : 47)];
+        ba[w] = g < 3 ? v : 0.f;
+      }
+    } else {
+#pragma unroll
+      for (int w = 0; w < 3; ++w) ba[w] = (active && g < 3) ? agg[(h * 3 + w) * 48 + lane] : 0.f;
+#pragma unroll
+      for (int w = 0; w < 3; ++w)
+#pragma unroll
+        for (int f = 0; f < 3; ++f)
+          xv[w][f] = (G::TAIL && active) ? agg[(h * 3 + w) * 48 + 16 * f + j] : 0.f;
+    }
+    f32x4 X[G::MT_D][3];
+#pragma unroll
+    for (int mt = 0; mt < G::MT_D; ++mt) {
+      const float aw = tab[G::T_TEW + mt * 64 + lane];
+#pragma unroll
+      for (int w = 0; w < 3; ++w) X[mt][w] = mfma(aw, ba[w], ld4(tab + G::T_TE + w * G::DP + 16 * mt + 4 * g));
+    }
+    static_assert(kLayers == 2, "layer 0 (folded q/k/v) + layer 1");
+    if constexpr (G::TAIL) {
+      encoder_layer_tail<H, true, SPLIT, AS>(X, ring, tab + G::T_L0, lane, tab, ba, xv);
+      encoder_layer_tail<H, false, SPLIT, AS>(X, ring, tab + G::T_L0 + G::TL_SIZE, lane, tab, ba, xv);
+    } else if constexpr (!SPLIT) {
+      encoder_layer<H, true>(X, ring, tab + G::T_L0, lane, tab, ba);
+      encoder_layer<H, false>(X, ring, tab + G::T_L0 + G::TL_SIZE, lane, tab, ba);
+    }
+
+    if (active) {
+#pragma unroll
+      for (int w = 0; w < 3; ++w) {
+        float* lc = lat + (long)((h * 3 + w) * G::KS_D) * 64;
+#pragma unroll
+        for (int q = 0; q < G::LAT_FG; ++q) *reinterpret_cast<f32x4*>(lc + q * 256 + lane * 4) = X[q][w];
+        if constexpr (G::KS_D % 4 != 0) {
+#pragma unroll
+          for (int r = 0; r < G::KS_D % 4; ++r) lc[G::LAT_FG * 256 + r * 64 + lane] = X[G::LAT_FG][w][r];
+        }
+      }
+      if (a.latent != nullptr) {
+        int jt = j, gt = g;
+        if constexpr (AS) asm volatile("" : "+v"(jt), "+v"(gt));
+        const long b = blk * 16 + jt;
+        if (b < a.B) {
+#pragma unroll
+          for (int w = 0; w < 3; ++w)
+#pragma unroll
+            for (int mt = 0; mt < G::MT_D; ++mt)
+#pragma unroll
+              for (int r = 0; r < 4; ++r) {
+                const int c = 16 * mt + 4 * r + gt;
+                const float* TL1 = tab + G::T_L0 + G::TL_SIZE;
+                if (c < H)
+                  a.latent[b * G::LAT + (long)h * 3 * H + w * H + c] =
+                      X[mt][w][r] * TL1[G::TL_LN2G + 16 * mt + 4 * gt + r] + TL1[G::TL_LN2B + 16 * mt + 4 * gt + r];
+              }
+        }
+      }
+    }
+  };
+  if constexpr (L::UNITS) {
+    const long U = nblk * H, NWT = (long)gridDim.x * NW, gw = (long)blockIdx.x * NW + wv;
+    const long u1 = (gw + 1) * U / NWT;
+    float* slot = xstage + wv * 144;
+    const long u0 = gw * U / NWT;
+    float pf[3];
+    auto load_x = [&](long u) {
+#pragma unroll
+      for (int k = 0; k < 3; ++k) pf[k] = a.agg[u * 144 + (64 * k + lane < 144 ? 64 * k + lane : 143)];
+    };
+    auto stage_x = [&]() {
+#pragma unroll
+      for (int k = 0; k < 3; ++k)
+        if (64 * k + lane < 144) slot[64 * k + lane] = pf[k];
+    };
+    if (u0 < u1) {
+      load_x(u0);
+      stage_x();
+    }
+#pragma unroll 1
+    for (long u = u0; u < u1; ++u) {
+      load_x(u + 1 < u1 ? u + 1 : u);
+      const long blk = u / H;
+      unit(blk, (int)(u - blk * H), true, slot);
+      stage_x();
+    }
+  } else {
+    const long blk = (long)blockIdx.x * NW + wv;
+    const bool active = blk < nblk;
+#pragma unroll 1
+    for (int h = 0; h < H; ++h) unit(blk, h, active, nullptr);
+  }
diff --git a/preganplus_amd/model.py b/preganplus_amd/model.py
--- a/preganplus_amd/model.py
+++ b/preganplus_amd/model.py
@@ -67,8 +67,8 @@
     def gan_split(self, on: bool):
         _native.check(self._L.pgp_gan_split(self._h, int(bool(on))), "pgp_gan_split")
 
-    def encoder_split(self, on: bool):
-        _native.check(self._L.pgp_encoder_split(self._h, int(bool(on))), "pgp_encoder_split")
+    def encoder_split(self, on):
+        _native.check(self._L.pgp_encoder_split(self._h, int(on)), "pgp_encoder_split")
 
     def decoder_split(self, on: bool):
         _native.check(self._L.pgp_decoder_split(self._h, int(bool(on))), "pgp_decoder_split")
diff --git a/preganplus_amd/roofline.py b/preganplus_amd/roofline.py
--- a/preganplus_amd/roofline.py
+++ b/preganplus_amd/roofline.py
@@ -55,8 +55,11 @@
     return H in ENC_SPLIT_MFMA_PER_HOST
 
 
+ENC_ASPLIT_MFMA_PER_HOST = {50: (48, 936)}
+
+
 def encoder_split_executed_flops_per_window(H: int):
-    f32, bf = ENC_SPLIT_MFMA_PER_HOST[H]
+    f32, bf = ENC_ASPLIT_MFMA_PER_HOST.get(H) or ENC_SPLIT_MFMA_PER_HOST[H]
     return f32 * 2048 * H / 16, bf * 16 * 16 * 32 * 2 * H / 16
 
 
```

New measurement: 706.5 million host-windows/s, median of 6. 9.2% higher.
